# PJLab-ADG/neuralsim

Hardware: NVIDIA H100
Metric: Mrays/sec fwd+bwd (higher is better)
Workload: dtype f16

## Files before the change

### neuralsim_b200/csrc/color_tc.cu

```cuda
#include "fused_tc_common.cuh"
#include "sh_device.cuh"

namespace nsb {

struct ColorNetDev {
    DecoderDevTC dec;
    const __half *R1, *rb1, *R2, *rb2, *R3, *rb3;
    int rw, rin, n_appear;
    float fac[3];
};

constexpr int XW = 64;
constexpr int kTileBytes = kTile * XW * 2;
constexpr int kChunk = kTile * 16;

__host__ __device__ inline int ref_col(int k, int n_appear) {
    if (k < 32) return 22 + k;
    if (k < 35) return k - 32;
    if (k < 51) return 3 + (k - 35);
    if (k < 54) return 19 + (k - 51);
    if (k < 54 + n_appear) return k;
    return -1;
}


__device__ __forceinline__ void level_jacobian(const PLMeta &m, uint32_t p, const float (&xs)[3], const __half *__restrict__ grid,
                                               float (&J0)[3], float (&J1)[3]) {
    uint32_t cell[8];
    float w[8], fr[3], scale[3];
    level_cells3(m, p, xs, cell, w, fr, scale);
    const uint32_t *lp = level_cells_ptr(m, p, grid);
    float2 v[8];
#pragma unroll
    for (int c = 0; c < 8; ++c) {
        const uint32_t raw = ld_nc_u32(lp + cell[c]);
        v[c] = __half22float2(*reinterpret_cast<const __half2 *>(&raw));
    }
#pragma unroll
    for (int gd = 0; gd < 3; ++gd) {
        float a0 = 0.f, a1 = 0.f;
#pragma unroll
        for (int c = 0; c < 4; ++c) {
            float ww = scale[gd];
            int left = 0;
#pragma unroll
            for (int k = 0; k < 2; ++k) {
                const int d = k >= gd ? k + 1 : k;
                if (c & (1 << k)) { ww = __fmul_rn(ww, fr[d]); left += 1 << d; }
                else ww = __fmul_rn(ww, __fsub_rn(1.f, fr[d]));
            }
            const int right = left + (1 << gd);
            a0 = __fmaf_rn(ww, __fsub_rn(v[right].x, v[left].x), a0);
            a1 = __fmaf_rn(ww, __fsub_rn(v[right].y, v[left].y), a1);
        }
        J0[gd] = a0;
        J1[gd] = a1;
    }
}

__device__ __forceinline__ void unpack8(const uint4 &q, float (&v)[8]) {
    const __half2 *h = reinterpret_cast<const __half2 *>(&q);
#pragma unroll
    for (int i = 0; i < 4; ++i) { const float2 f = __half22float2(h[i]); v[2 * i] = f.x; v[2 * i + 1] = f.y; }
}

constexpr int kColorGatherU = 4;

constexpr int kColorBwdCtasPerSM = 2;

__global__ void __launch_bounds__(kTile)
k_color_fwd(const PLMeta m, const __half *__restrict__ grid, const ColorNetDev net, const PointSrc ps, const float *__restrict__ view_dirs,
            const float *__restrict__ h_appear, int64_t n, int max_level, float *__restrict__ sdf_out, float *__restrict__ nab_out,
            float *__restrict__ rgb_out, float *__restrict__ x_out, uint8_t *__restrict__ Zt, uint8_t *__restrict__ Xt,
            uint8_t *__restrict__ Y1t, uint8_t *__restrict__ Y2t, const OccCollect oc, const int64_t *__restrict__ n_dev) {
    n = eff_n(n, n_dev);
    extern __shared__ uint8_t dyn_smem[];
    uint8_t *tiles = reinterpret_cast<uint8_t *>((reinterpret_cast<uintptr_t>(dyn_smem) + 1023) & ~uintptr_t(1023));
    uint8_t *sX = tiles;
    uint8_t *sU = sX + kTileBytes;
    uint8_t *sW1 = sU + kTileBytes;
    uint8_t *sW1T = sW1 + HW * NF * 2;
    uint8_t *sR1 = sW1T + HW * NF * 2;
    uint8_t *sR2 = sR1 + XW * XW * 2;
    constexpr int kS = tc::acc_stride(64);
    float *acc = reinterpret_cast<float *>(sR2 + XW * XW * 2);
    __shared__ float sb1[HW], sW2[HW], srb1[XW], srb2[XW], sR3[3][XW];
    __shared__ float sb2, srb3[3];

    const int tid = threadIdx.x;
    stage_W1(net.dec, sW1, tid);
    stage_W1T(net.dec, sW1T, tid);
    for (int e = tid; e < XW * XW; e += kTile) {
        const int j = e % XW, k = e / XW;
        const int rc = ref_col(k, net.n_appear);
        const __half v1 = (j < net.rw && rc >= 0) ? net.R1[j * net.rin + rc] : __float2half_rn(0.f);
        const __half v2 = (j < net.rw && k < net.rw) ? net.R2[j * net.rw + k] : __float2half_rn(0.f);
        *reinterpret_cast<__half *>(sR1 + (k / 8) * (XW * 16) + j * 16 + (k % 8) * 2) = v1;
        *reinterpret_cast<__half *>(sR2 + (k / 8) * (XW * 16) + j * 16 + (k % 8) * 2) = v2;
    }
    stage_decoder_vectors(net.dec, sb1, sW2, &sb2, tid);
    if (tid < XW) {
        srb1[tid] = tid < net.rw ? __half2float(net.rb1[tid]) : 0.f;
        srb2[tid] = tid < net.rw ? __half2float(net.rb2[tid]) : 0.f;
#pragma unroll
        for (int k = 0; k < 3; ++k) sR3[k][tid] = tid < net.rw ? __half2float(net.R3[k * net.rw + tid]) : 0.f;
    }
    if (tid == 0) {
        for (int k = 0; k < 3; ++k) srb3[k] = __half2float(net.rb3[k]);
    }
    tc::fence_async_smem();
    __syncthreads();
    const uint32_t x_addr = tc::smem_u32(sX), u_addr = tc::smem_u32(sU), w1_addr = tc::smem_u32(sW1), w1t_addr = tc::smem_u32(sW1T);
    const uint32_t r1_addr = tc::smem_u32(sR1), r2_addr = tc::smem_u32(sR2);
    const SoftplusK spk(net.dec.beta);

    const int64_t n_tiles = (n + kTile - 1) / kTile;
    for (int64_t tile = blockIdx.x; tile < n_tiles; tile += gridDim.x) {
        const int64_t i = tile * kTile + tid;
        const bool valid = i < n;
        float xn[3], xs[3];
        int64_t ray;
        load_point(ps, ps.x == nullptr, i, valid, xn, xs, ray);
        gather_row_to_tile<kTile, kColorGatherU>(m, grid, xs, max_level, sX, tid);
        tc::fence_async_smem();
        __syncthreads();
        tc::mma_to_rows<64, 0, 0, NF / 16>(acc, kS, 0, tc::kmajor(x_addr, kTile), tc::kmajor(w1_addr, HW), false);
        __syncthreads();
        float out = 0.f;
        uint8_t *zt = Zt ? Zt + tile * kTileBytes : nullptr;
#pragma unroll 1
        for (int c = 0; c < HW / 8; ++c) {
            float z[8], uu[8];
            tc::acc_ld8(acc, kS, tid, c * 8, z);
#pragma unroll
            for (int j = 0; j < 8; ++j) {
                z[j] = r16(z[j] + sb1[c * 8 + j]);
                float a, s;
                softplus_as(z[j], spk, a, s);
                out = fmaf(r16(a), sW2[c * 8 + j], out);
                uu[j] = sW2[c * 8 + j] * s;
            }
            *reinterpret_cast<uint4 *>(sU + c * kChunk + tid * 16) = tc::pack8_f16(uu);
            if (zt) *reinterpret_cast<uint4 *>(zt + c * kChunk + tid * 16) = tc::pack8_f16(z);
        }
        const float sdf = r16(out + sb2);
        tc::fence_async_smem();
        __syncthreads();
        tc::mma_to_rows<32, 0, 0, HW / 16>(acc, kS, 0, tc::kmajor(u_addr, kTile), tc::kmajor(w1t_addr, NF), false);
        __syncthreads();
        float nacc[3] = {0.f, 0.f, 0.f};
#pragma unroll 1
        for (uint32_t g4 = 0; g4 < 4; ++g4) {
            float gg[8];
            tc::acc_ld8(acc, kS, tid, g4 * 8, gg);
#pragma unroll
            for (uint32_t q = 0; q < 4; ++q) {
                const uint32_t p = g4 * 4 + q;
                if ((int)m.level[p] <= max_level) {
                    float J0[3], J1[3];
                    level_jacobian(m, p, xs, grid, J0, J1);
                    const float g0 = r16(gg[2 * q]), g1 = r16(gg[2 * q + 1]);
#pragma unroll
                    for (int d = 0; d < 3; ++d) nacc[d] = __fmaf_rn(g0, J0[d], nacc[d]);
#pragma unroll
                    for (int d = 0; d < 3; ++d) nacc[d] = __fmaf_rn(g1, J1[d], nacc[d]);
                }
            }
        }
        float nab[3];
#pragma unroll
        for (int d = 0; d < 3; ++d) nab[d] = __fmul_rn(__fmul_rn(nacc[d], 0.5f), net.fac[d]);
        {
            float xr[32];
#pragma unroll
            for (int k = 0; k < 32; ++k) xr[k] = 0.f;
            xr[0] = xn[0]; xr[1] = xn[1]; xr[2] = xn[2];
            if (valid) {
                sh_basis(view_dirs[ray * 3], view_dirs[ray * 3 + 1], view_dirs[ray * 3 + 2], 4, xr + 3);
                if (h_appear) {
#pragma unroll
                    for (int k = 0; k < 8; ++k)
                        if (k < net.n_appear) xr[22 + k] = h_appear[ray * net.n_appear + k];
                }
            }
#pragma unroll
            for (int d = 0; d < 3; ++d) xr[19 + d] = fminf(fmaxf(nab[d], -1.f), 1.f);
            uint8_t *xt = Xt ? Xt + tile * kTileBytes : nullptr;
#pragma unroll
            for (int c = 0; c < 4; ++c) {
                float v8[8];
#pragma unroll
                for (int k = 0; k < 8; ++k) v8[k] = xr[c * 8 + k];
                const uint4 q = tc::pack8_f16(v8);
                *reinterpret_cast<uint4 *>(sX + (4 + c) * kChunk + tid * 16) = q;
                if (xt) {
                    *reinterpret_cast<uint4 *>(xt + (4 + c) * kChunk + tid * 16) = q;
                    *reinterpret_cast<uint4 *>(xt + c * kChunk + tid * 16) = *reinterpret_cast<const uint4 *>(sX + c * kChunk + tid * 16);
                }
            }
        }
        tc::fence_async_smem();
        __syncthreads();
        tc::mma_to_rows<64, 0, 0, XW / 16>(acc, kS, 0, tc::kmajor(x_addr, kTile), tc::kmajor(r1_addr, XW), false);
        __syncthreads();
        uint8_t *y1t = Y1t ? Y1t + tile * kTileBytes : nullptr;
#pragma unroll 1
        for (int c = 0; c < XW / 8; ++c) {
            float y[8];
            tc::acc_ld8(acc, kS, tid, c * 8, y);
#pragma unroll
            for (int j = 0; j < 8; ++j) y[j] = fmaxf(r16(y[j] + srb1[c * 8 + j]), 0.f);
            const uint4 q = tc::pack8_f16(y);
            *reinterpret_cast<uint4 *>(sU + c * kChunk + tid * 16) = q;
            if (y1t) *reinterpret_cast<uint4 *>(y1t + c * kChunk + tid * 16) = q;
        }
        tc::fence_async_smem();
        __syncthreads();
        tc::mma_to_rows<64, 0, 0, XW / 16>(acc, kS, 0, tc::kmajor(u_addr, kTile), tc::kmajor(r2_addr, XW), false);
        __syncthreads();
        float o3[3] = {0.f, 0.f, 0.f};
        uint8_t *y2t = Y2t ? Y2t + tile * kTileBytes : nullptr;
#pragma unroll 1
        for (int c = 0; c < XW / 8; ++c) {
            float y[8];
            tc::acc_ld8(acc, kS, tid, c * 8, y);
#pragma unroll
            for (int j = 0; j < 8; ++j) {
                y[j] = fmaxf(r16(y[j] + srb2[c * 8 + j]), 0.f);
#pragma unroll
                for (int k = 0; k < 3; ++k) o3[k] = fmaf(y[j], sR3[k][c * 8 + j], o3[k]);
            }
            if (y2t) *reinterpret_cast<uint4 *>(y2t + c * kChunk + tid * 16) = tc::pack8_f16(y);
        }
        if (valid) {
            sdf_out[i] = sdf;
            if (oc.pcl) occ_collect_point(oc, xs, sdf);
#pragma unroll
            for (int d = 0; d < 3; ++d) {
                nab_out[i * 3 + d] = nab[d];
                const float y3 = r16(o3[d] + srb3[d]);
                rgb_out[i * 3 + d] = r16(1.f / (1.f + expf(-y3)));
                if (x_out) x_out[i * 3 + d] = xn[d];
            }
        }
        __syncthreads();
    }
}

__global__ void __launch_bounds__(kTile, kColorBwdCtasPerSM)
k_color_rad_bwd(const ColorNetDev net, const uint8_t *__restrict__ Xt, const uint8_t *__restrict__ Y1t, const uint8_t *__restrict__ Y2t,
                const float *__restrict__ rgb, const float *__restrict__ g_rgb, int64_t n, float *__restrict__ dh_out,
                float *__restrict__ dR1, float *__restrict__ drb1, float *__restrict__ dR2, float *__restrict__ drb2,
                float *__restrict__ dR3, float *__restrict__ drb3, const int64_t *__restrict__ n_dev) {
    n = eff_n(n, n_dev);
    constexpr int NE = 80;
    extern __shared__ uint8_t dyn_smem[];
    uint8_t *tiles = reinterpret_cast<uint8_t *>((reinterpret_cast<uintptr_t>(dyn_smem) + 1023) & ~uintptr_t(1023));
    uint8_t *sT = tiles;
    uint8_t *sY1 = sT + 3 * kTileBytes;
    uint8_t *sXe = sY1 + kTile * NE * 2;
    uint8_t *sR2T = sXe + kTile * NE * 2;
    uint8_t *sR1h = sR2T + XW * XW * 2;
    __shared__ float sR3[3][XW];
    __shared__ float sdb3[3];
    __shared__ __align__(8) uint64_t mbar_ld;

    const int tid = threadIdx.x, lane = tid & 31;
    for (int e = tid; e < XW * XW; e += kTile) {
        const int i = e % XW, j = e / XW;
        const __half v = (j < net.rw && i < net.rw) ? net.R2[j * net.rw + i] : __float2half_rn(0.f);
        *reinterpret_cast<__half *>(sR2T + (j / 8) * (XW * 16) + i * 16 + (j % 8) * 2) = v;
    }
    for (int e = tid; e < NF * XW; e += kTile) {
        const int k = e % NF, j = e / NF;
        const __half v = j < net.rw ? net.R1[j * net.rin + 22 + k] : __float2half_rn(0.f);
        *reinterpret_cast<__half *>(sR1h + (j / 8) * (NF * 16) + k * 16 + (j % 8) * 2) = v;
    }
    if (tid < XW) {
#pragma unroll
        for (int k = 0; k < 3; ++k) sR3[k][tid] = tid < net.rw ? __half2float(net.R3[k * net.rw + tid]) : 0.f;
    }
    *reinterpret_cast<uint4 *>(sY1 + 8 * kChunk + tid * 16) = make_uint4(0x00003C00u, 0, 0, 0);
    *reinterpret_cast<uint4 *>(sY1 + 9 * kChunk + tid * 16) = make_uint4(0, 0, 0, 0);
    *reinterpret_cast<uint4 *>(sXe + 9 * kChunk + tid * 16) = make_uint4(0, 0, 0, 0);
    float xa[NE / 2], xb[NE / 2], x3[4];
#pragma unroll
    for (int k = 0; k < NE / 2; ++k) xa[k] = xb[k] = 0.f;
#pragma unroll
    for (int k = 0; k < 4; ++k) x3[k] = 0.f;
    if (tid == 0) {
        sdb3[0] = sdb3[1] = sdb3[2] = 0.f;
        tc::mbar_init(&mbar_ld, 1);
        tc::fence_mbar_init();
    }
    tc::fence_async_smem();
    __syncthreads();
    const uint32_t t_addr = tc::smem_u32(sT), y1_addr = tc::smem_u32(sY1), xe_addr = tc::smem_u32(sXe);
    const uint32_t r2t_addr = tc::smem_u32(sR2T), r1h_addr = tc::smem_u32(sR1h);
    uint32_t ld_phase = 0;
    bool first_tile = true;

    const int64_t n_tiles = (n + kTile - 1) / kTile;
    auto fetch = [&](int64_t tile) {
        tc::mbar_arrive_expect_tx(&mbar_ld, 3 * kTileBytes);
        tc::tma_load_bulk(sT + 2 * kTileBytes, Y2t + tile * kTileBytes, kTileBytes, &mbar_ld);
        tc::tma_load_bulk(sY1, Y1t + tile * kTileBytes, kTileBytes, &mbar_ld);
        tc::tma_load_bulk(sXe, Xt + tile * kTileBytes, kTileBytes, &mbar_ld);
    };
    if (tid == 0 && (int64_t)blockIdx.x < n_tiles) fetch(blockIdx.x);
    for (int64_t tile = blockIdx.x; tile < n_tiles; tile += gridDim.x) {
        const int64_t i = tile * kTile + tid;
        const bool valid = i < n;
        tc::mbar_wait(&mbar_ld, ld_phase);
        ld_phase ^= 1;
        float gy[3] = {0.f, 0.f, 0.f};
        if (valid && g_rgb) {
#pragma unroll
            for (int k = 0; k < 3; ++k) {
                const float y = rgb[i * 3 + k];
                gy[k] = r16(r16(g_rgb[i * 3 + k]) * ((1.f - y) * y));
            }
        }
        {
            float e8[8] = {1.f, gy[0], gy[1], gy[2], 0.f, 0.f, 0.f, 0.f};
            *reinterpret_cast<uint4 *>(sXe + 8 * kChunk + tid * 16) = tc::pack8_f16(e8);
        }
#pragma unroll
        for (int k = 0; k < 3; ++k) {
            const float sgy = warp_sum(gy[k]);
            if (lane == 0 && sgy != 0.f) atomicAdd(&sdb3[k], sgy);
        }
#pragma unroll 1
        for (int c = 0; c < 8; ++c) {
            float y2[8], d[8];
            unpack8(*reinterpret_cast<const uint4 *>(sT + 2 * kTileBytes + c * kChunk + tid * 16), y2);
#pragma unroll
            for (int j = 0; j < 8; ++j) {
                const float v = gy[0] * sR3[0][c * 8 + j] + gy[1] * sR3[1][c * 8 + j] + gy[2] * sR3[2][c * 8 + j];
                d[j] = y2[j] > 0.f ? v : 0.f;
            }
            *reinterpret_cast<uint4 *>(sT + c * kChunk + tid * 16) = tc::pack8_f16(d);
        }
        tc::fence_async_smem();
        __syncthreads();
        {
            float dy[2][XW / 2];
            tc::mma_m128<64, 0, 0, XW / 16>(dy, tc::kmajor(t_addr, kTile), tc::kmajor(r2t_addr, XW), false);
#pragma unroll
            for (int h = 0; h < 2; ++h)
#pragma unroll
                for (int c = 0; c < XW / 8; ++c)
#pragma unroll
                    for (int r = 0; r < 2; ++r) {
                        const uint32_t off = tc::pair_off<kTile>(h * 64 + tc::frag_row(r), tc::frag_col(c));
                        const float2 y1 = tc::ld_pair_f16(sY1, off);
                        tc::st_pair_f16(sT + kTileBytes, off, y1.x > 0.f ? dy[h][4 * c + 2 * r] : 0.f, y1.y > 0.f ? dy[h][4 * c + 2 * r + 1] : 0.f);
                    }
        }
        tc::fence_async_smem();
        __syncthreads();
        float dh[2][NF / 2];
        tc::mma_m128<32, 0, 0, XW / 16>(dh, tc::kmajor(t_addr + kTileBytes, kTile), tc::kmajor(r1h_addr, NF), false);
        tc::mma_m64<NE, 1, 1, kTile / 16>(xa, tc::mnmajor(t_addr, kTile), tc::mnmajor(y1_addr, kTile), true);
        tc::mma_m64<NE, 1, 1, kTile / 16>(xb, tc::mnmajor(t_addr + kTileBytes, kTile), tc::mnmajor(xe_addr, kTile), true);
        tc::mma_m64<8, 1, 1, kTile / 16>(x3, tc::mnmajor(t_addr + 2 * kTileBytes, kTile), tc::mnmajor(xe_addr + 8 * kChunk, kTile), true);
        first_tile = false;
        __syncthreads();
        if (tid == 0 && tile + gridDim.x < n_tiles) {
            tc::fence_async_smem();
            fetch(tile + gridDim.x);
        }
#pragma unroll
        for (int h = 0; h < 2; ++h)
#pragma unroll
            for (int r = 0; r < 2; ++r) {
                const int64_t row = tile * kTile + h * 64 + tc::frag_row(r);
                if (row < n) {
#pragma unroll
                    for (int c = 0; c < NF / 8; ++c)
                        *reinterpret_cast<float2 *>(dh_out + row * NF + tc::frag_col(c)) = make_float2(dh[h][4 * c + 2 * r], dh[h][4 * c + 2 * r + 1]);
                }
            }
    }
    if (!first_tile) {
#pragma unroll
        for (int r = 0; r < 2; ++r) {
            const int row = tc::frag_row(r);
            if (row >= net.rw) continue;
#pragma unroll
            for (int c = 0; c < NE / 8; ++c)
#pragma unroll
                for (int j = 0; j < 2; ++j) {
                    const int col = tc::frag_col(c) + j;
                    const float a = xa[4 * c + 2 * r + j], b = xb[4 * c + 2 * r + j];
                    if (col < XW) {
                        if (col < net.rw) atomicAdd(dR2 + row * net.rw + col, a);
                        const int rc = ref_col(col, net.n_appear);
                        if (rc >= 0) atomicAdd(dR1 + row * net.rin + rc, b);
                    } else if (col == XW) {
                        atomicAdd(drb2 + row, a);
                        atomicAdd(drb1 + row, b);
                    }
                }
#pragma unroll
            for (int j = 0; j < 2; ++j) {
                const int col = tc::frag_col(0) + j;
                if (col >= 1 && col <= 3) atomicAdd(dR3 + (col - 1) * net.rw + row, x3[2 * r + j]);
            }
        }
        if (tid < 3) atomicAdd(drb3 + tid, sdb3[tid]);
    }
}

__global__ void __launch_bounds__(kTile, kColorBwdCtasPerSM)
k_color_sdf_bwd(const PLMeta m, const __half *__restrict__ grid, const ColorNetDev net, const PointSrc ps, const uint8_t *__restrict__ Zt,
                const uint8_t *__restrict__ Xt, const float *__restrict__ g_nab, const float *__restrict__ g_sdf, const float *__restrict__ dh_r,
                int64_t n, int max_level, float *__restrict__ d_grid, float *__restrict__ d_W1, float *__restrict__ d_b1, float *__restrict__ d_W2,
                float *__restrict__ d_b2, const int64_t *__restrict__ n_dev) {
    n = eff_n(n, n_dev);
    constexpr int NX = 48;
    extern __shared__ uint8_t dyn_smem[];
    uint8_t *tiles = reinterpret_cast<uint8_t *>((reinterpret_cast<uintptr_t>(dyn_smem) + 1023) & ~uintptr_t(1023));
    uint8_t *sT = tiles;
    uint8_t *sHe = sT + 3 * kTileBytes;
    uint8_t *sGe = sHe + kTile * NX * 2;
    uint8_t *sW1 = sGe + kTile * NX * 2;
    uint8_t *sW1T = sW1 + HW * NF * 2;
    uint8_t *sZ = sW1T + NF * HW * 2;
    constexpr int kS = tc::acc_stride(2 * NF);
    float *stage = reinterpret_cast<float *>(sT);
    static_assert(kTile * kS * 4 <= 3 * kTileBytes, "the staged rows must fit in T");
    __shared__ float sW2[HW], sdsdf[kTile];
    __shared__ float sdb2;
    __shared__ __align__(8) uint64_t mbar_ld;

    const int tid = threadIdx.x, lane = tid & 31;
    stage_W1(net.dec, sW1, tid);
    stage_W1T(net.dec, sW1T, tid);
    stage_decoder_vectors(net.dec, nullptr, sW2, nullptr, tid);
    *reinterpret_cast<uint4 *>(sHe + 4 * kChunk + tid * 16) = make_uint4(0x00003C00u, 0, 0, 0);
    *reinterpret_cast<uint4 *>(sGe + 4 * kChunk + tid * 16) = make_uint4(0x00003C00u, 0, 0, 0);
    *reinterpret_cast<uint4 *>(sHe + 5 * kChunk + tid * 16) = make_uint4(0, 0, 0, 0);
    *reinterpret_cast<uint4 *>(sGe + 5 * kChunk + tid * 16) = make_uint4(0, 0, 0, 0);
    float wacc[NX / 2], vacc[4];
#pragma unroll
    for (int k = 0; k < NX / 2; ++k) wacc[k] = 0.f;
#pragma unroll
    for (int k = 0; k < 4; ++k) vacc[k] = 0.f;
    if (tid == 0) {
        sdb2 = 0.f;
        tc::mbar_init(&mbar_ld, 1);
        tc::fence_mbar_init();
    }
    tc::fence_async_smem();
    __syncthreads();
    const uint32_t t_addr = tc::smem_u32(sT), he_addr = tc::smem_u32(sHe), ge_addr = tc::smem_u32(sGe), w1_addr = tc::smem_u32(sW1),
                   w1t_addr = tc::smem_u32(sW1T);
    const SoftplusK spk(net.dec.beta);
    uint32_t ld_phase = 0;
    bool first_tile = true;

    const int64_t n_tiles = (n + kTile - 1) / kTile;
    auto fetch = [&](int64_t tile) {
        tc::mbar_arrive_expect_tx(&mbar_ld, kTileBytes + 4 * kChunk);
        tc::tma_load_bulk(sZ, Zt + tile * kTileBytes, kTileBytes, &mbar_ld);
        tc::tma_load_bulk(sHe, Xt + tile * kTileBytes, 4 * kChunk, &mbar_ld);
    };
    if (tid == 0 && (int64_t)blockIdx.x < n_tiles) fetch(blockIdx.x);
    for (int64_t tile = blockIdx.x; tile < n_tiles; tile += gridDim.x) {
        const int64_t i = tile * kTile + tid;
        const bool valid = i < n;
        float xn[3], xs[3];
        int64_t ray;
        load_point(ps, ps.x == nullptr, i, valid, xn, xs, ray);
        float gin[3] = {0.f, 0.f, 0.f};
        if (valid && g_nab) {
#pragma unroll
            for (int d = 0; d < 3; ++d) gin[d] = g_nab[i * 3 + d] * net.fac[d] * 0.5f;
        }
        const float dsdf = (valid && g_sdf) ? g_sdf[i] : 0.f;
        sdsdf[tid] = dsdf;
        tc::mbar_wait(&mbar_ld, ld_phase);
        ld_phase ^= 1;
#pragma unroll 1
        for (int c = 0; c < 8; ++c) {
            float z[8], uu[8];
            unpack8(*reinterpret_cast<const uint4 *>(sZ + c * kChunk + tid * 16), z);
#pragma unroll
            for (int j = 0; j < 8; ++j) {
                float a, s;
                softplus_as(z[j], spk, a, s);
                uu[j] = sW2[c * 8 + j] * s;
            }
            *reinterpret_cast<uint4 *>(sT + kTileBytes + c * kChunk + tid * 16) = tc::pack8_f16(uu);
        }
#pragma unroll 4
        for (uint32_t p = 0; p < 16; ++p) {
            uint32_t packed = 0;
            if ((int)m.level[p] <= max_level) {
                float J0[3], J1[3];
                level_jacobian(m, p, xs, grid, J0, J1);
                float a0 = 0.f, a1 = 0.f;
#pragma unroll
                for (int d = 0; d < 3; ++d) { a0 = __fmaf_rn(gin[d], J0[d], a0); a1 = __fmaf_rn(gin[d], J1[d], a1); }
                const __half2 h = __floats2half2_rn(a0, a1);
                packed = *reinterpret_cast<const uint32_t *>(&h);
            }
            *reinterpret_cast<uint32_t *>(sGe + (p >> 2) * kChunk + tid * 16 + (p & 3) * 4) = packed;
        }
        tc::fence_async_smem();
        __syncthreads();
        float gfr[2][NF / 2];
        {
            float du[2][HW / 2];
            tc::mma_m128<64, 0, 0, NF / 16>(du, tc::kmajor(ge_addr, kTile), tc::kmajor(w1_addr, HW), false);
            tc::mma_m128<32, 0, 0, HW / 16>(gfr, tc::kmajor(t_addr + kTileBytes, kTile), tc::kmajor(w1t_addr, NF), false);
#pragma unroll
            for (int h = 0; h < 2; ++h)
#pragma unroll
                for (int r = 0; r < 2; ++r) {
                    const int row = h * 64 + tc::frag_row(r);
                    const float ds = sdsdf[row];
#pragma unroll
                    for (int c = 0; c < HW / 8; ++c) {
                        const int col = tc::frag_col(c);
                        const uint32_t off = tc::pair_off<kTile>(row, col);
                        const float2 z2 = tc::ld_pair_f16(sZ, off);
                        float dz[2], vv[2];
#pragma unroll
                        for (int j = 0; j < 2; ++j) {
                            const float z = j ? z2.y : z2.x;
                            float a, s;
                            softplus_as(z, spk, a, s);
                            const float w2 = sW2[col + j], d = r16(du[h][4 * c + 2 * r + j]);
                            const float curv = (z * spk.k > spk.thr) ? 0.f : spk.beta * s * (1.f - s);
                            dz[j] = d * w2 * curv + ds * w2 * s;
                            vv[j] = d * s + ds * r16(a);
                        }
                        tc::st_pair_f16(sT, off, dz[0], dz[1]);
                        tc::st_pair_f16(sT + 2 * kTileBytes, off, vv[0], vv[1]);
                    }
                }
        }
        tc::fence_async_smem();
        __syncthreads();
        float dhz[2][NF / 2];
        tc::mma_m128<32, 0, 0, HW / 16>(dhz, tc::kmajor(t_addr, kTile), tc::kmajor(w1t_addr, NF), false);
        tc::mma_m64<NX, 1, 1, kTile / 16>(wacc, tc::mnmajor(t_addr, kTile), tc::mnmajor(he_addr, kTile), true);
        tc::mma_m64<NF, 1, 1, kTile / 16>(*reinterpret_cast<float(*)[NF / 2]>(wacc), tc::mnmajor(t_addr + kTileBytes, kTile), tc::mnmajor(ge_addr, kTile), true);
        tc::mma_m64<8, 1, 1, kTile / 16>(vacc, tc::mnmajor(t_addr + 2 * kTileBytes, kTile), tc::mnmajor(ge_addr + 4 * kChunk, kTile), true);
        first_tile = false;
        const float dsum = warp_sum(dsdf);
        if (lane == 0 && dsum != 0.f) atomicAdd(&sdb2, dsum);
        __syncthreads();
        if (tid == 0 && tile + gridDim.x < n_tiles) {
            tc::fence_async_smem();
            fetch(tile + gridDim.x);
        }
        tc::frag_store<NF>(gfr, stage, kS, 0);
        tc::frag_store<NF>(dhz, stage, kS, NF);
        __syncthreads();
#pragma unroll 1
        for (uint32_t g4 = 0; g4 < 4; ++g4) {
            float gg[8], hz[8];
            tc::acc_ld8(stage, kS, tid, g4 * 8, gg);
            tc::acc_ld8(stage, kS, tid, NF + g4 * 8, hz);
            if (valid && dh_r) {
                const float4 r0 = *reinterpret_cast<const float4 *>(dh_r + i * NF + g4 * 8), r1 = *reinterpret_cast<const float4 *>(dh_r + i * NF + g4 * 8 + 4);
                hz[0] += r0.x; hz[1] += r0.y; hz[2] += r0.z; hz[3] += r0.w; hz[4] += r1.x; hz[5] += r1.y; hz[6] += r1.z; hz[7] += r1.w;
            }
#pragma unroll
            for (uint32_t q = 0; q < 4; ++q) {
                const uint32_t p = g4 * 4 + q;
                if ((int)m.level[p] > max_level) continue;
                uint32_t cell[8];
                float w[8], fr[3], sc[3], ua[8], ub[8];
                level_cells3(m, p, xs, cell, w, fr, sc);
                const float g0 = valid ? r16(gg[2 * q]) : 0.f, g1 = valid ? r16(gg[2 * q + 1]) : 0.f;
                const float h0 = valid ? hz[2 * q] : 0.f, h1 = valid ? hz[2 * q + 1] : 0.f;
#pragma unroll
                for (int c = 0; c < 8; ++c) {
                    float wsum = 0.f;
#pragma unroll
                    for (int gd = 0; gd < 3; ++gd) {
                        float ww = __fmul_rn(sc[gd], gin[gd]);
#pragma unroll
                        for (int d = 0; d < 3; ++d) {
                            if (d == gd) continue;
                            ww = __fmul_rn(ww, (c & (1 << d)) ? fr[d] : __fsub_rn(1.f, fr[d]));
                        }
                        wsum += (c & (1 << gd)) ? ww : -ww;
                    }
                    ua[c] = g0 * wsum + h0 * w[c];
                    ub[c] = g1 * wsum + h1 * w[c];
                }
                bool issue = valid;
                if (level_mergeable(m, p)) issue = warp_merge_updates(cell_key3(m, p, xs), valid, ua, ub, lane);
                if (issue) {
                    float2 *gp = level_grad_ptr(m, p, d_grid);
#pragma unroll
                    for (int c = 0; c < 8; ++c) red_add2(gp + cell[c], ua[c], ub[c]);
                }
            }
        }
        __syncthreads();
    }
    if (!first_tile) {
#pragma unroll
        for (int r = 0; r < 2; ++r) {
            const int row = tc::frag_row(r);
            if (row >= net.dec.width) continue;
#pragma unroll
            for (int c = 0; c <= NF / 8; ++c)
#pragma unroll
                for (int j = 0; j < 2; ++j) {
                    const int col = tc::frag_col(c) + j;
                    if (col < NF) atomicAdd(d_W1 + row * NF + col, wacc[4 * c + 2 * r + j]);
                    else if (col == NF) atomicAdd(d_b1 + row, wacc[4 * c + 2 * r + j]);
                }
            if (tc::frag_col(0) == 0) atomicAdd(d_W2 + row, vacc[2 * r]);
        }
        if (tid == 0) atomicAdd(d_b2, sdb2);
    }
}

}

using namespace nsb;

namespace {
int make_net(const nsb_color_net *c, const nsb_lotd_meta *meta, PLMeta *m, ColorNetDev *d, const char *who) {
    const nsb_sdf_decoder dec{c->W1, c->b1, c->W2, c->b2, c->width, c->beta};
    if (int rc = make_decoder(meta, &dec, m, &d->dec, who)) return rc;
    NSB_REQUIRE(c->rad_width >= 1 && c->rad_width <= 64, "%s: radiance width must be <= 64", who);
    NSB_REQUIRE(c->n_appear >= 0 && c->n_appear <= 8 && c->rad_in == 54 + c->n_appear,
                "%s: radiance input must be [x(3), SH deg 4 (16), n(3), h(32), h_appear(<=8)]", who);
    d->R1 = (const __half *)c->R1; d->rb1 = (const __half *)c->rb1; d->R2 = (const __half *)c->R2; d->rb2 = (const __half *)c->rb2;
    d->R3 = (const __half *)c->R3; d->rb3 = (const __half *)c->rb3;
    d->rw = c->rad_width; d->rin = c->rad_in; d->n_appear = c->n_appear;
    for (int k = 0; k < 3; ++k) d->fac[k] = c->nablas_scale[k];
    return 0;
}
}

static int64_t n_tiles(int64_t n) { return (n + kTile - 1) / kTile; }

extern "C" int64_t nsb_color_tile_bytes(int64_t n) { return n_tiles(n) * (int64_t)kTileBytes; }

extern "C" int nsb_fused_color_fwd(const nsb_lotd_meta *meta, const void *params_half, const nsb_color_net *net, const float *x, const float *rays_o,
                                   const float *rays_d, const int64_t *ridx, const float *t, const float *view_dirs, const float *h_appear,
                                   int64_t n, int32_t max_level, float *sdf, float *nablas, float *rgb, float *x_out, void *act_z, void *act_x,
                                   void *act_y1, void *act_y2, const nsb_occ_collect *collect, void *stream) {
    const DevCounts dn = take_counts();
    if (n == 0) return 0;
    NSB_REQUIRE(meta && params_half && net && sdf && nablas && rgb && view_dirs, "nsb_fused_color_fwd: NULL argument");
    NSB_REQUIRE(x || (rays_o && rays_d && t), "nsb_fused_color_fwd: need x or (rays_o, rays_d, t)");
    NSB_REQUIRE((act_z && act_x && act_y1 && act_y2) || (!act_z && !act_x && !act_y1 && !act_y2), "nsb_fused_color_fwd: pass all four activation buffers or none");
    PLMeta m;
    ColorNetDev d;
    if (int rc = make_net(net, meta, &m, &d, "nsb_fused_color_fwd")) return rc;
    NSB_REQUIRE(d.n_appear == 0 || h_appear, "nsb_fused_color_fwd: h_appear is NULL but the net has %d appearance channels", d.n_appear);
    constexpr int kSmem = 2 * kTileBytes + 2 * HW * NF * 2 + 2 * XW * XW * 2 + kTile * tc::acc_stride(64) * 4 + 1024;
    opt_in_smem(k_color_fwd, kSmem);
    const PointSrc ps{x, rays_o, rays_d, t, ridx};
    k_color_fwd<<<persistent_grid(n_tiles(n), 2), kTile, kSmem, (cudaStream_t)stream>>>(m, (const __half *)params_half, d, ps, view_dirs, h_appear, n,
                                                                                        max_level < 0 ? -1 : max_level, sdf, nablas, rgb, x_out, (uint8_t *)act_z,
                                                                                        (uint8_t *)act_x, (uint8_t *)act_y1, (uint8_t *)act_y2,
                                                                                        occ_collect_of(collect), dn.a);
    return check_launch("nsb_fused_color_fwd");
}

extern "C" int nsb_fused_color_bwd(const nsb_lotd_meta *meta, const void *params_half, const nsb_color_net *net, const float *x, const float *rays_o,
                                   const float *rays_d, const int64_t *ridx, const float *t, int64_t n, int32_t max_level, const void *act_z,
                                   const void *act_x, const void *act_y1, const void *act_y2, const float *rgb, const float *g_sdf,
                                   const float *g_nablas, const float *g_rgb, float *dh_scratch, float *d_grid, float *d_W1, float *d_b1,
                                   float *d_W2, float *d_b2, float *d_R1, float *d_rb1, float *d_R2, float *d_rb2, float *d_R3, float *d_rb3,
                                   void *stream) {
    const DevCounts dn = take_counts();
    if (n == 0) return 0;
    NSB_REQUIRE(meta && params_half && net && act_z && act_x && act_y1 && act_y2 && rgb && dh_scratch, "nsb_fused_color_bwd: NULL argument");
    NSB_REQUIRE(d_grid && d_W1 && d_b1 && d_W2 && d_b2 && d_R1 && d_rb1 && d_R2 && d_rb2 && d_R3 && d_rb3, "nsb_fused_color_bwd: NULL gradient buffer");
    NSB_REQUIRE(x || (rays_o && rays_d && t), "nsb_fused_color_bwd: need x or (rays_o, rays_d, t)");
    PLMeta m;
    ColorNetDev d;
    if (int rc = make_net(net, meta, &m, &d, "nsb_fused_color_bwd")) return rc;
    cudaStream_t s = (cudaStream_t)stream;
    const float *dh = nullptr;
    if (g_rgb) {
        constexpr int kSmemR = 3 * kTileBytes + 2 * kTile * 80 * 2 + XW * XW * 2 + NF * XW * 2 + 1024;
        opt_in_smem(k_color_rad_bwd, kSmemR);
        if (int rc = require_ctas_per_sm(k_color_rad_bwd, kTile, kSmemR, kColorBwdCtasPerSM, "nsb_fused_color_bwd(radiance)")) return rc;
        k_color_rad_bwd<<<persistent_grid(n_tiles(n), kColorBwdCtasPerSM), kTile, kSmemR, s>>>(d, (const uint8_t *)act_x, (const uint8_t *)act_y1,
                                                                                               (const uint8_t *)act_y2, rgb, g_rgb, n, dh_scratch, d_R1,
                                                                                               d_rb1, d_R2, d_rb2, d_R3, d_rb3, dn.a);
        if (int rc = check_launch("nsb_fused_color_bwd(radiance)")) return rc;
        dh = dh_scratch;
    }
    constexpr int kSmemS = 3 * kTileBytes + 2 * kTile * 48 * 2 + 2 * HW * NF * 2 + kTileBytes + 1024;
    opt_in_smem(k_color_sdf_bwd, kSmemS);
    if (int rc = require_ctas_per_sm(k_color_sdf_bwd, kTile, kSmemS, kColorBwdCtasPerSM, "nsb_fused_color_bwd(sdf)")) return rc;
    const PointSrc ps{x, rays_o, rays_d, t, ridx};
    k_color_sdf_bwd<<<persistent_grid(n_tiles(n), kColorBwdCtasPerSM), kTile, kSmemS, s>>>(m, (const __half *)params_half, d, ps, (const uint8_t *)act_z, (const uint8_t *)act_x,
                                                                          g_nablas, g_sdf, dh, n, max_level < 0 ? -1 : max_level, d_grid, d_W1, d_b1, d_W2, d_b2, dn.a);
    return check_launch("nsb_fused_color_bwd(sdf)");
}
```

### neuralsim_b200/csrc/tc_util.cuh

```cuda
#pragma once
#include "nsb_common.cuh"

namespace nsb {
namespace tc {

__device__ __forceinline__ uint32_t smem_u32(const void *p) { return (uint32_t)__cvta_generic_to_shared(p); }

__device__ __forceinline__ uint64_t make_desc(uint32_t smem_addr, uint32_t lbo_bytes, uint32_t sbo_bytes) {
    uint64_t d = 0;
    d |= (uint64_t)((smem_addr >> 4) & 0x3FFF);
    d |= (uint64_t)((lbo_bytes >> 4) & 0x3FFF) << 16;
    d |= (uint64_t)((sbo_bytes >> 4) & 0x3FFF) << 32;
    return d;
}

struct Operand {
    uint32_t addr, lbo, sbo, kstep;
};
__device__ __forceinline__ Operand kmajor(uint32_t addr, int rows) { return Operand{addr, (uint32_t)rows * 16, 128, (uint32_t)rows * 32}; }
__device__ __forceinline__ Operand mnmajor(uint32_t addr, int rows) { return Operand{addr, 128, (uint32_t)rows * 16, 256}; }

template <int N, int TA, int TB>
struct Wgmma;
template <int TA, int TB>
struct Wgmma<8, TA, TB> {
    __device__ __forceinline__ static void mma(float (&d)[4], uint64_t a, uint64_t b, uint32_t acc) {
        asm volatile(
            "{\n\t.reg .pred p;\n\tsetp.ne.b32 p, %6, 0;\n\t"
            "wgmma.mma_async.sync.aligned.m64n8k16.f32.f16.f16 {%0, %1, %2, %3}, %4, %5, p, 1, 1, %7, %8;\n\t}\n"
            : "+f"(d[0]), "+f"(d[1]), "+f"(d[2]), "+f"(d[3])
            : "l"(a), "l"(b), "r"(acc), "n"(TA), "n"(TB));
    }
};
template <int TA, int TB>
struct Wgmma<32, TA, TB> {
    __device__ __forceinline__ static void mma(float (&d)[16], uint64_t a, uint64_t b, uint32_t acc) {
        asm volatile(
            "{\n\t.reg .pred p;\n\tsetp.ne.b32 p, %18, 0;\n\t"
            "wgmma.mma_async.sync.aligned.m64n32k16.f32.f16.f16 {%0, %1, %2, %3, %4, %5, %6, %7, %8, %9, %10, %11, %12, %13, %14, %15}, %16, %17, p, 1, 1, %19, %20;\n\t}\n"
            : "+f"(d[0]), "+f"(d[1]), "+f"(d[2]), "+f"(d[3]), "+f"(d[4]), "+f"(d[5]), "+f"(d[6]), "+f"(d[7]), "+f"(d[8]), "+f"(d[9]), "+f"(d[10]), "+f"(d[11]), "+f"(d[12]), "+f"(d[13]), "+f"(d[14]), "+f"(d[15])
            : "l"(a), "l"(b), "r"(acc), "n"(TA), "n"(TB));
    }
};
template <int TA, int TB>
struct Wgmma<40, TA, TB> {
    __device__ __forceinline__ static void mma(float (&d)[20], uint64_t a, uint64_t b, uint32_t acc) {
        asm volatile(
            "{\n\t.reg .pred p;\n\tsetp.ne.b32 p, %22, 0;\n\t"
            "wgmma.mma_async.sync.aligned.m64n40k16.f32.f16.f16 {%0, %1, %2, %3, %4, %5, %6, %7, %8, %9, %10, %11, %12, %13, %14, %15, %16, %17, %18, %19}, %20, %21, p, 1, 1, %23, %24;\n\t}\n"
            : "+f"(d[0]), "+f"(d[1]), "+f"(d[2]), "+f"(d[3]), "+f"(d[4]), "+f"(d[5]), "+f"(d[6]), "+f"(d[7]), "+f"(d[8]), "+f"(d[9]), "+f"(d[10]), "+f"(d[11]), "+f"(d[12]), "+f"(d[13]), "+f"(d[14]), "+f"(d[15]), "+f"(d[16]), "+f"(d[17]), "+f"(d[18]), "+f"(d[19])
            : "l"(a), "l"(b), "r"(acc), "n"(TA), "n"(TB));
    }
};
template <int TA, int TB>
struct Wgmma<48, TA, TB> {
    __device__ __forceinline__ static void mma(float (&d)[24], uint64_t a, uint64_t b, uint32_t acc) {
        asm volatile(
            "{\n\t.reg .pred p;\n\tsetp.ne.b32 p, %26, 0;\n\t"
            "wgmma.mma_async.sync.aligned.m64n48k16.f32.f16.f16 {%0, %1, %2, %3, %4, %5, %6, %7, %8, %9, %10, %11, %12, %13, %14, %15, %16, %17, %18, %19, %20, %21, %22, %23}, %24, %25, p, 1, 1, %27, %28;\n\t}\n"
            : "+f"(d[0]), "+f"(d[1]), "+f"(d[2]), "+f"(d[3]), "+f"(d[4]), "+f"(d[5]), "+f"(d[6]), "+f"(d[7]), "+f"(d[8]), "+f"(d[9]), "+f"(d[10]), "+f"(d[11]), "+f"(d[12]), "+f"(d[13]), "+f"(d[14]), "+f"(d[15]), "+f"(d[16]), "+f"(d[17]), "+f"(d[18]), "+f"(d[19]), "+f"(d[20]), "+f"(d[21]), "+f"(d[22]), "+f"(d[23])
            : "l"(a), "l"(b), "r"(acc), "n"(TA), "n"(TB));
    }
};
template <int TA, int TB>
struct Wgmma<64, TA, TB> {
    __device__ __forceinline__ static void mma(float (&d)[32], uint64_t a, uint64_t b, uint32_t acc) {
        asm volatile(
            "{\n\t.reg .pred p;\n\tsetp.ne.b32 p, %34, 0;\n\t"
            "wgmma.mma_async.sync.aligned.m64n64k16.f32.f16.f16 {%0, %1, %2, %3, %4, %5, %6, %7, %8, %9, %10, %11, %12, %13, %14, %15, %16, %17, %18, %19, %20, %21, %22, %23, %24, %25, %26, %27, %28, %29, %30, %31}, %32, %33, p, 1, 1, %35, %36;\n\t}\n"
            : "+f"(d[0]), "+f"(d[1]), "+f"(d[2]), "+f"(d[3]), "+f"(d[4]), "+f"(d[5]), "+f"(d[6]), "+f"(d[7]), "+f"(d[8]), "+f"(d[9]), "+f"(d[10]), "+f"(d[11]), "+f"(d[12]), "+f"(d[13]), "+f"(d[14]), "+f"(d[15]), "+f"(d[16]), "+f"(d[17]), "+f"(d[18]), "+f"(d[19]), "+f"(d[20]), "+f"(d[21]), "+f"(d[22]), "+f"(d[23]), "+f"(d[24]), "+f"(d[25]), "+f"(d[26]), "+f"(d[27]), "+f"(d[28]), "+f"(d[29]), "+f"(d[30]), "+f"(d[31])
            : "l"(a), "l"(b), "r"(acc), "n"(TA), "n"(TB));
    }
};
template <int TA, int TB>
struct Wgmma<80, TA, TB> {
    __device__ __forceinline__ static void mma(float (&d)[40], uint64_t a, uint64_t b, uint32_t acc) {
        asm volatile(
            "{\n\t.reg .pred p;\n\tsetp.ne.b32 p, %42, 0;\n\t"
            "wgmma.mma_async.sync.aligned.m64n80k16.f32.f16.f16 {%0, %1, %2, %3, %4, %5, %6, %7, %8, %9, %10, %11, %12, %13, %14, %15, %16, %17, %18, %19, %20, %21, %22, %23, %24, %25, %26, %27, %28, %29, %30, %31, %32, %33, %34, %35, %36, %37, %38, %39}, %40, %41, p, 1, 1, %43, %44;\n\t}\n"
            : "+f"(d[0]), "+f"(d[1]), "+f"(d[2]), "+f"(d[3]), "+f"(d[4]), "+f"(d[5]), "+f"(d[6]), "+f"(d[7]), "+f"(d[8]), "+f"(d[9]), "+f"(d[10]), "+f"(d[11]), "+f"(d[12]), "+f"(d[13]), "+f"(d[14]), "+f"(d[15]), "+f"(d[16]), "+f"(d[17]), "+f"(d[18]), "+f"(d[19]), "+f"(d[20]), "+f"(d[21]), "+f"(d[22]), "+f"(d[23]), "+f"(d[24]), "+f"(d[25]), "+f"(d[26]), "+f"(d[27]), "+f"(d[28]), "+f"(d[29]), "+f"(d[30]), "+f"(d[31]), "+f"(d[32]), "+f"(d[33]), "+f"(d[34]), "+f"(d[35]), "+f"(d[36]), "+f"(d[37]), "+f"(d[38]), "+f"(d[39])
            : "l"(a), "l"(b), "r"(acc), "n"(TA), "n"(TB));
    }
};

__device__ __forceinline__ void wgmma_fence() { asm volatile("wgmma.fence.sync.aligned;" ::: "memory"); }
__device__ __forceinline__ void wgmma_commit() { asm volatile("wgmma.commit_group.sync.aligned;" ::: "memory"); }
__device__ __forceinline__ void wgmma_wait_all() { asm volatile("wgmma.wait_group.sync.aligned 0;" ::: "memory"); }
__device__ __forceinline__ void fence_operand(float &r) { asm volatile("" : "+f"(r)::"memory"); }

template <int N, int TA, int TB, int KSTEPS>
__device__ __forceinline__ void mma_m128(float (&d)[2][N / 2], const Operand &a, const Operand &b, bool accumulate) {
#pragma unroll
    for (int h = 0; h < 2; ++h)
#pragma unroll
        for (int i = 0; i < N / 2; ++i) fence_operand(d[h][i]);
    wgmma_fence();
#pragma unroll
    for (int h = 0; h < 2; ++h)
#pragma unroll
        for (int ks = 0; ks < KSTEPS; ++ks)
            Wgmma<N, TA, TB>::mma(d[h], make_desc(a.addr + h * 8 * a.sbo + ks * a.kstep, a.lbo, a.sbo), make_desc(b.addr + ks * b.kstep, b.lbo, b.sbo),
                                  (ks > 0 || accumulate) ? 1u : 0u);
    wgmma_commit();
    wgmma_wait_all();
#pragma unroll
    for (int h = 0; h < 2; ++h)
#pragma unroll
        for (int i = 0; i < N / 2; ++i) fence_operand(d[h][i]);
}

template <int N, int TA, int TB, int KSTEPS>
__device__ __forceinline__ void mma_m64(float (&d)[N / 2], const Operand &a, const Operand &b, bool accumulate) {
#pragma unroll
    for (int i = 0; i < N / 2; ++i) fence_operand(d[i]);
    wgmma_fence();
#pragma unroll
    for (int ks = 0; ks < KSTEPS; ++ks)
        Wgmma<N, TA, TB>::mma(d, make_desc(a.addr + ks * a.kstep, a.lbo, a.sbo), make_desc(b.addr + ks * b.kstep, b.lbo, b.sbo),
                              (ks > 0 || accumulate) ? 1u : 0u);
    wgmma_commit();
    wgmma_wait_all();
#pragma unroll
    for (int i = 0; i < N / 2; ++i) fence_operand(d[i]);
}

__device__ __forceinline__ int frag_row(int i) { return (threadIdx.x >> 5) * 16 + ((threadIdx.x & 31) >> 2) + 8 * i; }
__device__ __forceinline__ int frag_col(int c) { return c * 8 + 2 * (threadIdx.x & 3); }
template <int R>
__device__ __forceinline__ uint32_t pair_off(int row, int col) { return (uint32_t)((col >> 3) * (R * 16) + row * 16 + (col & 7) * 2); }
__device__ __forceinline__ float2 ld_pair_f16(const uint8_t *tile, uint32_t off) {
    return __half22float2(*reinterpret_cast<const __half2 *>(tile + off));
}
__device__ __forceinline__ void st_pair_f16(uint8_t *tile, uint32_t off, float a, float b) {
    *reinterpret_cast<__half2 *>(tile + off) = __floats2half2_rn(a, b);
}

constexpr int acc_stride(int cols) { return cols + 4; }

template <int N>
__device__ __forceinline__ void frag_store(const float (&d)[2][N / 2], float *acc, int stride, int col0) {
    const int w = threadIdx.x >> 5, l = threadIdx.x & 31;
#pragma unroll
    for (int h = 0; h < 2; ++h)
#pragma unroll
        for (int c = 0; c < N / 8; ++c)
#pragma unroll
            for (int i = 0; i < 2; ++i) {
                const int row = h * 64 + w * 16 + (l >> 2) + 8 * i, col = col0 + c * 8 + 2 * (l & 3);
                *reinterpret_cast<float2 *>(acc + row * stride + col) = make_float2(d[h][4 * c + 2 * i], d[h][4 * c + 2 * i + 1]);
            }
}
template <int N>
__device__ __forceinline__ void frag_load(float (&d)[2][N / 2], const float *acc, int stride, int col0) {
    const int w = threadIdx.x >> 5, l = threadIdx.x & 31;
#pragma unroll
    for (int h = 0; h < 2; ++h)
#pragma unroll
        for (int c = 0; c < N / 8; ++c)
#pragma unroll
            for (int i = 0; i < 2; ++i) {
                const int row = h * 64 + w * 16 + (l >> 2) + 8 * i, col = col0 + c * 8 + 2 * (l & 3);
                const float2 v = *reinterpret_cast<const float2 *>(acc + row * stride + col);
                d[h][4 * c + 2 * i] = v.x;
                d[h][4 * c + 2 * i + 1] = v.y;
            }
}
template <int N, int TA, int TB, int KSTEPS>
__device__ __forceinline__ void mma_to_rows(float *acc, int stride, int col0, const Operand &a, const Operand &b, bool accumulate) {
    float d[2][N / 2];
    if (accumulate) frag_load<N>(d, acc, stride, col0);
    else {
#pragma unroll
        for (int h = 0; h < 2; ++h)
#pragma unroll
            for (int i = 0; i < N / 2; ++i) d[h][i] = 0.f;
    }
    mma_m128<N, TA, TB, KSTEPS>(d, a, b, accumulate);
    frag_store<N>(d, acc, stride, col0);
}

__device__ __forceinline__ void acc_ld8(const float *acc, int stride, int row, int col, float (&v)[8]) {
    const float4 a = *reinterpret_cast<const float4 *>(acc + row * stride + col), b = *reinterpret_cast<const float4 *>(acc + row * stride + col + 4);
    v[0] = a.x; v[1] = a.y; v[2] = a.z; v[3] = a.w; v[4] = b.x; v[5] = b.y; v[6] = b.z; v[7] = b.w;
}

__device__ __forceinline__ void mbar_init(uint64_t *bar, uint32_t count) {
    asm volatile("mbarrier.init.shared::cta.b64 [%0], %1;" ::"r"(smem_u32(bar)), "r"(count) : "memory");
}
__device__ __forceinline__ void mbar_wait(uint64_t *bar, uint32_t parity) {
    asm volatile(
        "{\n\t.reg .pred p;\n\tWAIT_%=:\n\t"
        "mbarrier.try_wait.parity.shared::cta.b64 p, [%0], %1;\n\t"
        "@p bra DONE_%=;\n\tbra WAIT_%=;\n\tDONE_%=:\n\t}\n" ::"r"(smem_u32(bar)),
        "r"(parity)
        : "memory");
}

__device__ __forceinline__ void mbar_arrive_expect_tx(uint64_t *bar, uint32_t bytes) {
    asm volatile("mbarrier.arrive.expect_tx.shared::cta.b64 _, [%0], %1;" ::"r"(smem_u32(bar)), "r"(bytes) : "memory");
}
__device__ __forceinline__ void tma_load_bulk(void *smem_dst, const void *gmem_src, uint32_t bytes, uint64_t *bar) {
    asm volatile("cp.async.bulk.shared::cluster.global.mbarrier::complete_tx::bytes [%0], [%1], %2, [%3];" ::"r"(smem_u32(smem_dst)), "l"(gmem_src),
                 "r"(bytes), "r"(smem_u32(bar))
                 : "memory");
}

__device__ __forceinline__ void fence_async_smem() { asm volatile("fence.proxy.async.shared::cta;" ::: "memory"); }
__device__ __forceinline__ void fence_mbar_init() { asm volatile("fence.mbarrier_init.release.cluster;" ::: "memory"); }

__device__ __forceinline__ uint4 pack8_f16(const float (&v)[8]) {
    __half2 h0 = __floats2half2_rn(v[0], v[1]), h1 = __floats2half2_rn(v[2], v[3]);
    __half2 h2 = __floats2half2_rn(v[4], v[5]), h3 = __floats2half2_rn(v[6], v[7]);
    uint4 q;
    q.x = *reinterpret_cast<uint32_t *>(&h0); q.y = *reinterpret_cast<uint32_t *>(&h1);
    q.z = *reinterpret_cast<uint32_t *>(&h2); q.w = *reinterpret_cast<uint32_t *>(&h3);
    return q;
}

template <int R, int K>
__device__ __forceinline__ void store_row_f16(uint8_t *tile, int r, const float *vals) {
#pragma unroll
    for (int c = 0; c < K / 8; ++c) {
        __half2 h0 = __floats2half2_rn(vals[c * 8 + 0], vals[c * 8 + 1]);
        __half2 h1 = __floats2half2_rn(vals[c * 8 + 2], vals[c * 8 + 3]);
        __half2 h2 = __floats2half2_rn(vals[c * 8 + 4], vals[c * 8 + 5]);
        __half2 h3 = __floats2half2_rn(vals[c * 8 + 6], vals[c * 8 + 7]);
        uint4 q;
        q.x = *reinterpret_cast<uint32_t *>(&h0);
        q.y = *reinterpret_cast<uint32_t *>(&h1);
        q.z = *reinterpret_cast<uint32_t *>(&h2);
        q.w = *reinterpret_cast<uint32_t *>(&h3);
        *reinterpret_cast<uint4 *>(tile + c * (R * 16) + r * 16) = q;
    }
}

}
}
```

### neuralsim_b200/fields/fused_color.py

```python
from __future__ import annotations

import ctypes

import torch
from torch import autograd

from .. import _lib as L


class _FusedColor(autograd.Function):
    @staticmethod
    def forward(ctx, model, pts, view_dirs, h_appear, max_level, keep, collect, *params):
        grid16, net, _held = model._fused_color_state()
        ridx, t, rays_o, rays_d = pts
        n, dev = t.numel(), t.device
        meta = model.implicit_surface.encoding.meta
        sdf = torch.empty(n, dtype=torch.float32, device=dev)
        nab = torch.empty(n, 3, dtype=torch.float32, device=dev)
        rgb = torch.empty(n, 3, dtype=torch.float32, device=dev)
        x = torch.empty(n, 3, dtype=torch.float32, device=dev)
        acts = None
        if keep:
            acts = torch.empty(4, int(L.lib().nsb_color_tile_bytes(L.c_i64(n))), dtype=torch.uint8, device=dev)
        ap = [L.ptr(acts[k]) if keep else None for k in range(4)]
        with L.KERNEL_TIMER.time("fused_color_fwd", n):
            L.check(L.lib().nsb_fused_color_fwd(meta.c_ref, L.ptr(grid16, "f16"), ctypes.byref(net), None, L.ptr(rays_o, "f32"), L.ptr(rays_d, "f32"),
                                                L.ptr(ridx, "i64"), L.ptr(t, "f32"), L.ptr(view_dirs, "f32"), L.ptr(h_appear, "f32", allow_none=True),
                                                L.c_i64(n), L.c_i32(max_level), L.ptr(sdf), L.ptr(nab), L.ptr(rgb), L.ptr(x), *ap,
                                                ctypes.byref(collect) if collect is not None else None, L.stream_ptr()),
                    "fused_color_fwd")
        ctx.model, ctx.pts, ctx.max_level, ctx.n = model, pts, max_level, n
        ctx.held = (grid16, net, _held, acts, rgb)
        ctx.shapes = [p.shape for p in params]
        ctx.set_materialize_grads(False)
        ctx.mark_non_differentiable(x)
        return sdf, nab, rgb, x

    @staticmethod
    @autograd.function.once_differentiable
    def backward(ctx, g_sdf, g_nab, g_rgb, _gx):
        grid16, net, _held, acts, rgb = ctx.held
        if acts is None:
            raise RuntimeError("fused_color: backward through a forward that ran without grad")
        dev, n = rgb.device, ctx.n
        meta = ctx.model.implicit_surface.encoding.meta
        sizes = [int(torch.Size(s).numel()) for s in ctx.shapes[1:]]
        small = torch.zeros(sum(sizes), dtype=torch.float32, device=dev)
        grads, o = [torch.zeros(ctx.shapes[0], dtype=torch.float32, device=dev)], 0
        for sh, k in zip(ctx.shapes[1:], sizes):
            grads.append(small[o:o + k].view(sh))
            o += k
        if g_sdf is None and g_nab is None and g_rgb is None:
            return (None,) * 7 + tuple(grads)
        ridx, t, rays_o, rays_d = ctx.pts
        c = lambda g: None if g is None else g.contiguous().float()
        g_sdf, g_nab, g_rgb = c(g_sdf), c(g_nab), c(g_rgb)
        dh = torch.empty(n, 32, dtype=torch.float32, device=dev)
        with L.KERNEL_TIMER.time("fused_color_bwd", n):
            L.check(L.lib().nsb_fused_color_bwd(meta.c_ref, L.ptr(grid16, "f16"), ctypes.byref(net), None, L.ptr(rays_o, "f32"), L.ptr(rays_d, "f32"),
                                                L.ptr(ridx, "i64"), L.ptr(t, "f32"), L.c_i64(n), L.c_i32(ctx.max_level), L.ptr(acts[0]), L.ptr(acts[1]),
                                                L.ptr(acts[2]), L.ptr(acts[3]), L.ptr(rgb), L.ptr(g_sdf, allow_none=True), L.ptr(g_nab, allow_none=True),
                                                L.ptr(g_rgb, allow_none=True), L.ptr(dh), *[L.ptr(g) for g in grads], L.stream_ptr()),
                    "fused_color_bwd")
        return (None,) * 7 + tuple(grads)


def fused_color(model, ridx, t, rays_o, rays_d, view_dirs, h_appear=None, *, nablas_has_grad=True, collect=None):
    s, r = model.implicit_surface, model.radiance_net.blocks.layers
    d = s.decoder.layers
    params = (s.encoding.flattened_params, d[0].weight, d[0].bias, d[1].weight, d[1].bias, r[0].weight, r[0].bias, r[1].weight, r[1].bias,
              r[2].weight, r[2].bias)
    pts = (ridx.reshape(-1).contiguous().long(), t.detach().reshape(-1).contiguous().float(), rays_o.detach().contiguous().float(),
           rays_d.detach().contiguous().float())
    keep = torch.is_grad_enabled() and any(p.requires_grad for p in params)
    ha = None if h_appear is None else h_appear.detach().contiguous().float()
    sdf, nab, rgb, x = _FusedColor.apply(model, pts, view_dirs.detach().contiguous().float(), ha, s._ml(model.max_level), keep, collect, *params)
    if not nablas_has_grad:
        nab = nab.detach()
    return dict(sdf=sdf, nablas=nab, rgb=rgb, x=x)
```

### neuralsim_b200/graphics/neus_static.py

```python
from __future__ import annotations

import ctypes

import torch
import torch.nn.functional as F

from .. import _lib as L
from .raysample import batch_sample_step_linear
from .pack_ops import get_pack_infos_from_batch
from . import neus_fused as NF

__all__ = ["render_static", "StaticFrame", "CNT_SLOTS"]

CNT_SLOTS = dict(n_rays=0, pairs=2, marched_raw=3, hit_raw=4, kept_raw=6, kept_rays_raw=7, nonzero=9, marched=12, hit=13, fine0=14,
                 boundary=18, kept=19, overflow=20, kept_rays=21, merged0=22, rays_if_kept_fits=26, row_len=27)
_NULL = ctypes.c_void_p(0)
MARCH_ONEPASS = "auto"
MARCH_ONEPASS_MAX_BYTES = 64 << 20


def march_onepass(n_rays, max_steps):
    if MARCH_ONEPASS == "0":
        return False
    return MARCH_ONEPASS == "1" or 4 * int(n_rays) * int(max_steps) <= MARCH_ONEPASS_MAX_BYTES


def _slot(cnt, k):
    return ctypes.c_void_p(cnt.data_ptr() + 8 * k)


def _call(fn, what, cnt, k0, k1, *args):
    lib = L.lib()
    lib.nsb_bind_device_counts(_slot(cnt, k0), _slot(cnt, k1) if k1 is not None else _NULL)
    try:
        rc = fn(*args)
    finally:
        lib.nsb_bind_device_counts(_NULL, _NULL)
    L.check(rc, what)


def _scan(counts, cnt, slot, *, first=None, info2=None, index=None, pack=None, src=None, nz_src=None, ws=None):
    if ws is None:
        ws = torch.zeros(NF._scan_ws_bytes(), dtype=torch.uint8, device=counts.device)
    P = L.ptr
    L.check(L.lib().nsb_scan_counts(P(counts, "i32"), L.c_i64(counts.shape[0]), P(first, allow_none=True), P(info2, allow_none=True),
                                    P(index, allow_none=True), P(pack, allow_none=True), P(src, "i64", allow_none=True), P(nz_src, allow_none=True),
                                    _slot(cnt, slot), None, L.c_i64(0), P(ws), L.stream_ptr()), "scan_counts")


def _query_counts(cnt, phase, n_coarse1, num_fine, march_cap, kept_cap):
    nf = (ctypes.c_int32 * max(len(num_fine), 1))(*[int(n) for n in num_fine])
    L.check(L.lib().nsb_query_counts(ctypes.c_void_p(cnt.data_ptr()), L.c_i32(phase), L.c_i32(n_coarse1), nf, L.c_i32(len(num_fine)),
                                     L.c_i64(march_cap), L.c_i64(kept_cap), L.stream_ptr()), "query_counts")


def _sdf_launch(meta, grid16, dec, rays_o, rays_d, t, sdf, *, ridx=None, packs=None, ml, collect, cnt, slot, timer="lotd_gather"):
    P = L.ptr
    mode = 2 if packs is not None else 1
    with L.KERNEL_TIMER.time(timer, t.numel()):
        _call(L.lib().nsb_fused_sdf_collect, "fused_sdf", cnt, slot, None,
              meta.c_ref, P(grid16, "f16"), ctypes.byref(dec), None, P(rays_o, "f32"), P(rays_d, "f32"),
              P(ridx, "i64") if mode == 1 else None, P(t, "f32"), L.c_i64(t.numel()),
              P(packs[0], "i64") if mode == 2 else None, P(packs[1], "i64", allow_none=True) if mode == 2 else None,
              P(packs[2], "i64", allow_none=True) if mode == 2 and len(packs) > 2 else None,
              L.c_i64(packs[0].shape[0] if mode == 2 else 0), L.c_i32(mode), L.c_i32(ml), P(sdf),
              ctypes.byref(collect) if collect is not None else None, L.stream_ptr())
    return sdf


def _block_order(rays_inds, via, n_rays, cnt, slot):
    n = rays_inds.shape[0] if via is None else via.shape[0]
    order = torch.empty(n, dtype=torch.int64, device=rays_inds.device)
    _call(L.lib().nsb_ray_block_order, "ray_block_order", cnt, slot, None, L.ptr(rays_inds, "i64"), L.ptr(via, "i64", allow_none=True), L.c_i64(n),
          L.c_i64(n_rays), _slot(cnt, CNT_SLOTS["pairs"]), _slot(cnt, CNT_SLOTS["row_len"]), L.ptr(order), L.stream_ptr())
    return order


class _StaticSDF(torch.autograd.Function):

    @staticmethod
    def forward(ctx, st, ridx, t, packs, count_slot, grid, W1, b1, W2, b2):
        sdf = torch.empty(t.numel(), dtype=torch.float32, device=t.device)
        _sdf_launch(st.meta, st.grid16, st.dec, st.rays_o, st.rays_d, t, sdf, ridx=ridx if packs is None else None, packs=packs, ml=st.ml,
                    collect=st.collect, cnt=st.cnt, slot=count_slot, timer="fused_sdf_fwd")
        ctx.st, ctx.ridx, ctx.t = st, ridx, t
        ctx.shapes = (grid.shape, W1.shape, b1.shape, W2.shape, b2.shape)
        return sdf

    @staticmethod
    @torch.autograd.function.once_differentiable
    def backward(ctx, d_sdf):
        st, dev = ctx.st, d_sdf.device
        gs, w1s, b1s, w2s, b2s = ctx.shapes
        d_grid = torch.zeros(gs, dtype=torch.float32, device=dev)
        ks = [int(torch.Size(x).numel()) for x in (w1s, b1s, w2s, b2s)]
        small = torch.zeros(sum(ks), dtype=torch.float32, device=dev)
        d_W1, d_b1 = small[:ks[0]].view(w1s), small[ks[0]:ks[0] + ks[1]].view(b1s)
        d_W2, d_b2 = small[ks[0] + ks[1]:ks[0] + ks[1] + ks[2]].view(w2s), small[ks[0] + ks[1] + ks[2]:].view(b2s)
        d_sdf = d_sdf.contiguous().float()
        n = d_sdf.numel()
        P, cnt = L.ptr, st.cnt
        flag = torch.empty(n, dtype=torch.int32, device=dev)
        _call(L.lib().nsb_flag_nonzero, "flag_nonzero", cnt, CNT_SLOTS["boundary"], None, P(d_sdf, "f32"), L.c_i64(n), P(flag), L.stream_ptr())
        keep = torch.empty(n, dtype=torch.int64, device=dev)
        _scan(flag, cnt, CNT_SLOTS["nonzero"], index=keep, ws=st.ws[3])
        with L.KERNEL_TIMER.time("fused_sdf_bwd", n):
            _call(L.lib().nsb_fused_sdf_bwd_indexed, "fused_sdf_bwd", cnt, CNT_SLOTS["nonzero"], None,
                  st.meta.c_ref, P(st.grid16, "f16"), ctypes.byref(st.dec), None, P(st.rays_o, "f32"), P(st.rays_d, "f32"), P(ctx.ridx, "i64"),
                  P(ctx.t, "f32"), P(d_sdf, "f32"), P(keep, "i64"), L.c_i64(n), L.c_i32(st.ml), P(d_grid), P(d_W1), P(d_b1), P(d_W2), P(d_b2),
                  L.stream_ptr())
        return None, None, None, None, None, d_grid, d_W1, d_b1, d_W2, d_b2


class _StaticAlpha(torch.autograd.Function):

    @staticmethod
    def forward(ctx, sdf, inv_s, pack_infos, cnt, early_stop_eps, alpha_thre):
        sdf_c, inv_c = sdf.detach().contiguous().float(), inv_s.detach().contiguous().float().reshape(1)
        Pn, dev = pack_infos.shape[0], sdf_c.device
        alpha = torch.empty_like(sdf_c)
        sel = torch.empty(sdf_c.shape[0], dtype=torch.bool, device=dev)
        steps = torch.empty(Pn, dtype=torch.int32, device=dev)
        P = L.ptr
        _call(L.lib().nsb_neus_alpha_forward, "neus_alpha_forward", cnt, CNT_SLOTS["n_rays"], None, P(sdf_c, "f32"), P(pack_infos, "i64"), L.c_i64(Pn),
              P(inv_c, "f32"), L.c_f32(early_stop_eps), L.c_f32(alpha_thre), P(alpha), P(sel), P(steps), L.stream_ptr())
        ctx.save_for_backward(sdf_c, inv_c, pack_infos)
        ctx.cnt, ctx.inv_shape = cnt, inv_s.shape
        ctx.mark_non_differentiable(sel, steps)
        return alpha, sel, steps

    @staticmethod
    def backward(ctx, g_alpha, _gs, _gn):
        sdf_c, inv_c, pack_infos = ctx.saved_tensors
        g = g_alpha.contiguous().float()
        d_sdf = torch.empty_like(sdf_c)
        d_inv = torch.zeros(1, device=sdf_c.device, dtype=torch.float32)
        P = L.ptr
        _call(L.lib().nsb_neus_alpha_backward, "neus_alpha_backward", ctx.cnt, CNT_SLOTS["n_rays"], None, P(sdf_c, "f32"), P(pack_infos, "i64"),
              L.c_i64(pack_infos.shape[0]), P(inv_c, "f32"), P(g, "f32"), P(d_sdf), P(d_inv), L.stream_ptr())
        return (d_sdf if ctx.needs_input_grad[0] else None, d_inv.reshape(ctx.inv_shape) if ctx.needs_input_grad[1] else None, None, None, None, None)


class _StaticGather(torch.autograd.Function):

    @staticmethod
    def forward(ctx, src, pidx, gathered, cnt):
        ctx.save_for_backward(pidx)
        ctx.n, ctx.cnt = src.shape[0], cnt
        return gathered

    @staticmethod
    def backward(ctx, g):
        pidx, = ctx.saved_tensors
        g = g.contiguous().float()
        d = torch.zeros(ctx.n, dtype=torch.float32, device=g.device)
        P = L.ptr
        _call(L.lib().nsb_scatter_f32, "scatter_f32", ctx.cnt, CNT_SLOTS["kept"], None, P(g, "f32"), P(pidx, "i64"), L.c_i64(pidx.shape[0]), P(d), L.stream_ptr())
        return d, None, None, None


class _StaticColor(torch.autograd.Function):

    @staticmethod
    def forward(ctx, st, ridx, t, view_dirs, h_appear, keep_acts, *params):
        n, dev = t.numel(), t.device
        sdf = torch.empty(n, dtype=torch.float32, device=dev)
        nab = torch.empty(n, 3, dtype=torch.float32, device=dev)
        rgb = torch.empty(n, 3, dtype=torch.float32, device=dev)
        x = torch.empty(n, 3, dtype=torch.float32, device=dev)
        acts = torch.empty(4, int(L.lib().nsb_color_tile_bytes(L.c_i64(n))), dtype=torch.uint8, device=dev) if keep_acts else None
        ap = [L.ptr(acts[k]) if keep_acts else None for k in range(4)]
        P = L.ptr
        with L.KERNEL_TIMER.time("fused_color_fwd", n):
            _call(L.lib().nsb_fused_color_fwd, "fused_color_fwd", st.cnt, CNT_SLOTS["kept"], None,
                  st.meta.c_ref, P(st.grid16, "f16"), ctypes.byref(st.net), None, P(st.rays_o, "f32"), P(st.rays_d, "f32"), P(ridx, "i64"), P(t, "f32"),
                  P(view_dirs, "f32"), P(h_appear, "f32", allow_none=True), L.c_i64(n), L.c_i32(st.ml), P(sdf), P(nab), P(rgb), P(x), *ap,
                  ctypes.byref(st.collect) if st.collect is not None else None, L.stream_ptr())
        ctx.st, ctx.ridx, ctx.t, ctx.n = st, ridx, t, n
        ctx.held = (acts, rgb)
        ctx.shapes = [p.shape for p in params]
        ctx.set_materialize_grads(False)
        ctx.mark_non_differentiable(x)
        return sdf, nab, rgb, x

    @staticmethod
    @torch.autograd.function.once_differentiable
    def backward(ctx, g_sdf, g_nab, g_rgb, _gx):
        acts, rgb = ctx.held
        if acts is None:
            raise RuntimeError("static colour query: backward through a forward that ran without grad")
        st, dev, n = ctx.st, rgb.device, ctx.n
        sizes = [int(torch.Size(s).numel()) for s in ctx.shapes[1:]]
        small = torch.zeros(sum(sizes), dtype=torch.float32, device=dev)
        grads, o = [torch.zeros(ctx.shapes[0], dtype=torch.float32, device=dev)], 0
        for sh, k in zip(ctx.shapes[1:], sizes):
            grads.append(small[o:o + k].view(sh))
            o += k
        if g_sdf is None and g_nab is None and g_rgb is None:
            return (None,) * 6 + tuple(grads)
        c = lambda g: None if g is None else g.contiguous().float()
        g_sdf, g_nab, g_rgb = c(g_sdf), c(g_nab), c(g_rgb)
        dh = torch.empty(n, 32, dtype=torch.float32, device=dev)
        P = L.ptr
        with L.KERNEL_TIMER.time("fused_color_bwd", n):
            _call(L.lib().nsb_fused_color_bwd, "fused_color_bwd", st.cnt, CNT_SLOTS["kept"], None,
                  st.meta.c_ref, P(st.grid16, "f16"), ctypes.byref(st.net), None, P(st.rays_o, "f32"), P(st.rays_d, "f32"), P(ctx.ridx, "i64"),
                  P(ctx.t, "f32"), L.c_i64(n), L.c_i32(st.ml), P(acts[0]), P(acts[1]), P(acts[2]), P(acts[3]), P(rgb), P(g_sdf, allow_none=True),
                  P(g_nab, allow_none=True), P(g_rgb, allow_none=True), P(dh), *[P(g) for g in grads], L.stream_ptr())
        return (None,) * 6 + tuple(grads)


class _StaticComposite(torch.autograd.Function):

    @staticmethod
    def forward(ctx, alpha, t, rgb, nablas, pack_infos, ray_index, n_rays, cnt, normalize_depth, early_stop_eps, alpha_thre):
        a, tt = alpha.detach().contiguous().float(), t.detach().contiguous().float()
        r = None if rgb is None else rgb.detach().contiguous().float()
        nb = None if nablas is None else nablas.detach().contiguous().float()
        Pn, dev = pack_infos.shape[0], a.device
        vw = torch.empty_like(a)
        cols = 2 + (3 if r is not None else 0) + (3 if nb is not None else 0)
        buf = torch.zeros(cols * n_rays, device=dev)
        mask, depth = buf[:n_rays], buf[n_rays:2 * n_rays]
        rgb_o = buf[2 * n_rays:5 * n_rays].view(n_rays, 3) if r is not None else None
        o3 = 5 * n_rays if r is not None else 2 * n_rays
        nab_o = buf[o3:o3 + 3 * n_rays].view(n_rays, 3) if nb is not None else None
        P = L.ptr
        _call(L.lib().nsb_composite_forward, "composite_forward", cnt, CNT_SLOTS["kept_rays"], None, P(a, "f32"), P(tt, "f32"), P(r, "f32", allow_none=True),
              P(nb, "f32", allow_none=True), P(pack_infos, "i64"), L.c_i64(Pn), L.c_f32(early_stop_eps), L.c_f32(alpha_thre),
              ctypes.c_int(1 if normalize_depth else 0), P(ray_index, "i64"), P(vw), P(mask), P(depth), P(rgb_o, allow_none=True),
              P(nab_o, allow_none=True), L.stream_ptr())
        ctx.save_for_backward(a, tt, r, nb, vw, pack_infos, mask, depth, ray_index)
        ctx.cfg = (normalize_depth, early_stop_eps, alpha_thre, cnt)
        ctx.set_materialize_grads(False)
        empty = a.new_empty(0)
        return vw, mask, depth, (rgb_o if rgb_o is not None else empty), (nab_o if nab_o is not None else empty)

    @staticmethod
    def backward(ctx, g_vw, g_mask, g_depth, g_rgb, g_nab):
        a, tt, r, nb, vw, pack_infos, mask, depth, ray_index = ctx.saved_tensors
        normalize_depth, eps, thre, cnt = ctx.cfg

        def opt(g, present=True):
            return None if (g is None or not present) else g.contiguous().float()
        g_vw, g_mask, g_depth = opt(g_vw), opt(g_mask), opt(g_depth)
        g_rgb, g_nab = opt(g_rgb, r is not None), opt(g_nab, nb is not None)
        d_alpha = torch.empty_like(a)
        d_rgb = torch.empty_like(r) if r is not None else None
        d_nab = torch.empty_like(nb) if nb is not None else None
        P = L.ptr
        _call(L.lib().nsb_composite_backward, "composite_backward", cnt, CNT_SLOTS["kept_rays"], None,
              P(a, "f32"), P(tt, "f32"), P(r, allow_none=True), P(nb, allow_none=True), P(vw, "f32"), P(pack_infos, "i64"), L.c_i64(pack_infos.shape[0]),
              L.c_f32(eps), L.c_f32(thre), ctypes.c_int(1 if normalize_depth else 0), P(mask), P(depth), P(g_mask, allow_none=True),
              P(g_depth, allow_none=True), P(g_rgb, allow_none=True), P(g_nab, allow_none=True), P(g_vw, allow_none=True), P(ray_index, "i64"),
              P(d_alpha), P(d_rgb, allow_none=True), P(d_nab, allow_none=True), L.stream_ptr())
        return (d_alpha, None, d_rgb, d_nab) + (None,) * 7


class _State:
    __slots__ = ("meta", "grid16", "dec", "net", "held", "rays_o", "rays_d", "ml", "collect", "cnt", "ws")


def _fp16_images(model):
    s, b = model.implicit_surface, model.radiance_net.blocks.layers
    d = s.decoder.layers
    ps = [s.encoding.flattened_params, d[0].weight, d[0].bias, d[1].weight, d[1].bias, b[0].weight, b[0].bias, b[1].weight, b[1].bias, b[2].weight, b[2].bias]
    t = [torch.empty(p.shape, dtype=torch.half, device=p.device) for p in ps]
    with torch.no_grad():
        t[0].copy_(ps[0].detach())
        torch._foreach_copy_(t[1:], [p.detach() for p in ps[1:]])
    dec = L.SdfDecoderC(t[1].data_ptr(), t[2].data_ptr(), t[3].data_ptr(), t[4].data_ptr(), d[0].out_features, float(d[0].activation.beta))
    r3 = s.radius3d_original
    fk = (r3.data_ptr(), r3._version, float(s.sdf_scale))
    if getattr(model, "_fac_cache", (None,))[0] != fk:
        model._fac_cache = (fk, (s.sdf_scale / r3).float().tolist())
    net = L.ColorNetC(*[x.data_ptr() for x in t[1:]], d[0].out_features, b[0].out_features, b[0].in_features, b[0].in_features - 54,
                      float(d[0].activation.beta), (ctypes.c_float * 3)(*model._fac_cache[1]))
    return t, dec, net, ps


def static_supported(model, cfg):
    qp = dict(model.ray_query_cfg.get("query_param", {}) or {})
    occ = getattr(getattr(model, "accel", None), "occ", None)
    return (getattr(model, "_color_fusable", lambda: False)() and model.use_view_dirs and occ is not None and occ.occ_grid.dim() == 3
            and occ.occ_grid.numel() * 4 // 32 <= 96 * 1024 and qp.get("num_coarse", 0) > 0 and len(qp.get("upsample_inv_s_factors", (1, 4, 16))) <= 4
            and qp.get("coarse_step_cfg", {}).get("step_mode", "linear") == "linear" and (cfg.get("with_rgb", True) or cfg.get("with_normal", True)))


def render_static(model, rays_o, rays_d, rays_h_appear=None, *, near=None, far=None, march_cap, kept_cap, coherent=False, with_rgb=True, with_normal=True,
                  perturb=False, training=None, depth_use_normalized_vw=True, cnt=None):
    P, lib = L.ptr, L.lib()
    if perturb:
        raise RuntimeError("render_static: perturb=True is not built (random streams of capacity-sized draws differ from the reference's); "
                           "use the host-sized path (SingleVolumeRenderer.render)")
    training = model.training if training is None else training
    R, dev = rays_o.shape[0], rays_o.device
    qp = dict(model.ray_query_cfg.get("query_param", {}) or {})
    nc1 = int(qp["num_coarse"]) + 1
    factors = list(qp.get("upsample_inv_s_factors", (1, 4, 16)))
    n_stage = len(factors)
    num_fine = qp.get("num_fine", 8)
    num_fine = [num_fine] * n_stage if isinstance(num_fine, int) else list(num_fine)
    num_fine = [n // 2 * 2 + 1 for n in num_fine]
    nf_tot = int(sum(num_fine))
    upsample_inv_s = qp.get("upsample_inv_s", 64.) / model.upsample_s_divisor
    use_est = bool(qp.get("upsample_use_estimate_alpha", False))
    nablas_has_grad = bool(qp.get("nablas_has_grad", False))
    mc = dict(qp.get("march_cfg", {}))
    fac = mc.pop("step_size_factor", 1.0)
    step_size, dt_gamma = mc.get("step_size", 1e-3) * fac, mc.get("dt_gamma", 0.0) * fac
    max_steps, max_step_size = int(mc.get("max_steps", 512)), mc.get("max_step_size", 1e10)
    march_cap, kept_cap = int(march_cap), int(kept_cap)
    S_cap = R * (nc1 + nf_tot)
    if cnt is None:
        cnt = torch.zeros(32, dtype=torch.int64, device=dev)
    else:
        cnt.zero_()
    st = _State()
    st.cnt = cnt
    wsb = (NF._scan_ws_bytes() + 255) // 256 * 256
    st.ws = torch.zeros(4, wsb, dtype=torch.uint8, device=dev)
    with torch.no_grad():
        t16, st.dec, st.net, masters = _fp16_images(model)
        st.held, st.grid16 = t16, t16[0]
        st.meta = model.implicit_surface.encoding.meta
        st.ml = model.implicit_surface._ml(model.max_level)
        st.collect = model.accel.occ.collect_struct() if training else None
        sp = model.space
        if getattr(sp, "_host_cr", None) is None or sp._host_cr[0] != (sp.aabb.data_ptr(), sp.aabb._version):
            c, r = sp.center.tolist(), sp.radius3d.tolist()
            sp._host_cr = ((sp.aabb.data_ptr(), sp.aabb._version), (ctypes.c_float * 3)(*c), (ctypes.c_float * 3)(*r))
        o_n, d_n = torch.empty(R, 3, device=dev), torch.empty(R, 3, device=dev)
        nr, fr = torch.empty(R, device=dev), torch.empty(R, device=dev)
        flag = torch.empty(R, dtype=torch.int32, device=dev)
        L.check(lib.nsb_ray_test_aabb(P(rays_o.contiguous(), "f32"), P(rays_d.contiguous(), "f32"), L.c_i64(R), sp._host_cr[1], sp._host_cr[2],
                                      ctypes.c_int(0 if near is None else 1), L.c_f32(0. if near is None else near),
                                      ctypes.c_int(0 if far is None else 1), L.c_f32(0. if far is None else far), P(o_n), P(d_n), P(nr), P(fr), P(flag),
                                      _slot(cnt, CNT_SLOTS["pairs"]), _slot(cnt, CNT_SLOTS["row_len"]), L.stream_ptr()), "ray_test_aabb")
        rays_inds = torch.empty(R, dtype=torch.int64, device=dev)
        _scan(flag, cnt, CNT_SLOTS["n_rays"], index=rays_inds, ws=st.ws[0])
        order_b = _block_order(rays_inds, None, R, cnt, CNT_SLOTS["n_rays"]) if coherent else None
        ha = rays_h_appear.detach().contiguous().float() if (rays_h_appear is not None and model.use_h_appear) else None
        if ha is None and model.use_h_appear:
            ha = torch.zeros(R, model.radiance_net.blocks.layers[0].in_features - 54, device=dev)
        n_ha = ha.shape[1] if ha is not None else 0
        rbuf = torch.zeros(R * (8 + n_ha), device=dev)
        o_c, d_c = rbuf[:3 * R].view(R, 3), rbuf[3 * R:6 * R].view(R, 3)
        n_c, f_c = rbuf[6 * R:7 * R], rbuf[7 * R:8 * R]
        ha_c = rbuf[8 * R:].view(R, n_ha) if ha is not None else None
        _call(lib.nsb_gather_rays, "gather_rays", cnt, CNT_SLOTS["n_rays"], None, P(rays_inds, "i64"), L.c_i64(R), P(o_n), P(d_n), P(nr), P(fr), P(o_c), P(d_c),
              P(n_c), P(f_c), P(ha, allow_none=True), P(ha_c, allow_none=True), L.c_i32(0 if ha is None else ha.shape[1]), L.stream_ptr())
        st.rays_o, st.rays_d = o_c, d_c
        view_dirs = (d_c / d_c.norm(dim=-1).clamp_min(1.0e-10).unsqueeze(-1)).contiguous()
        coarse = batch_sample_step_linear(n_c, f_c, nc1, prefix_shape=[R], perturb=perturb).contiguous()
        occ_grid = model.accel.occ.occ_grid
        res = occ_grid.shape[-3:]
        g8 = occ_grid.contiguous().view(torch.uint8)
        bits = torch.empty((occ_grid.numel() + 31) // 32, dtype=torch.int32, device=dev)
        L.check(lib.nsb_pack_occ_bits(P(g8, "u8"), L.c_i64(occ_grid.numel()), P(bits), L.stream_ptr()), "pack_occ_bits")
        roi = torch.tensor([-1, -1, -1, 1, 1, 1], dtype=torch.float32, device=dev) if getattr(model, "_static_roi", None) is None else model._static_roi
        model._static_roi = roi
        margs = (L.c_i64(R), P(o_c, "f32"), P(d_c, "f32"), P(n_c, "f32"), P(f_c, "f32"), P(roi, "f32"), None, L.c_i32(res[0]), L.c_i32(res[1]), L.c_i32(res[2]),
                 P(g8, "u8"), L.c_f32(step_size), L.c_f32(max_step_size), L.c_f32(dt_gamma), ctypes.c_uint32(max_steps))
        num_steps = torch.empty(R, dtype=torch.int32, device=dev)
        rec_t = torch.empty(R * max_steps, dtype=torch.float32, device=dev) if march_onepass(R, max_steps) else None
        with L.KERNEL_TIMER.time("march", R):
            if rec_t is not None:
                _call(lib.nsb_ray_marching_record, "ray_marching_record", cnt, CNT_SLOTS["n_rays"], None, L.c_i64(R), P(o_c, "f32"), P(d_c, "f32"), P(n_c, "f32"),
                      P(f_c, "f32"), P(roi, "f32"), L.c_i32(res[0]), L.c_i32(res[1]), L.c_i32(res[2]), P(g8, "u8"), L.c_f32(step_size), L.c_f32(max_step_size),
                      L.c_f32(dt_gamma), ctypes.c_uint32(max_steps), P(num_steps), P(rec_t), P(bits), L.stream_ptr())
            else:
                _call(lib.nsb_ray_marching_listed, "ray_marching", cnt, CNT_SLOTS["n_rays"], None, *margs, None, P(num_steps), None, None, None, None, None, None,
                      L.c_i64(0), P(bits), L.stream_ptr())
        info2 = torch.empty(R, 2, dtype=torch.int32, device=dev)
        ridx_hit = torch.empty(R, dtype=torch.int64, device=dev)
        pack_infos = torch.empty(R, 2, dtype=torch.int64, device=dev)
        _scan(num_steps, cnt, CNT_SLOTS["marched_raw"], info2=info2, index=ridx_hit, pack=pack_infos, ws=st.ws[1])
        _query_counts(cnt, 0, nc1, num_fine, march_cap, kept_cap)
        depth = torch.empty(march_cap, dtype=torch.float32, device=dev)
        ridx32 = torch.empty(march_cap, dtype=torch.int32, device=dev)
        with L.KERNEL_TIMER.time("march", R):
            if rec_t is not None:
                _call(lib.nsb_march_compact, "march_compact", cnt, CNT_SLOTS["hit"], None, P(rec_t, "f32"), ctypes.c_uint32(max_steps), P(info2, "i32"),
                      P(ridx_hit, "i64"), L.c_i64(R), P(depth), P(ridx32), L.stream_ptr())
            else:
                _call(lib.nsb_ray_marching_listed, "ray_marching", cnt, CNT_SLOTS["hit"], None, *margs, P(info2), None, P(depth), None, P(ridx32), None, None,
                      P(ridx_hit, "i64"), L.c_i64(R), P(bits), L.stream_ptr())
        ridx = ridx32.long()
        from . import neus as GN
        fine_stages = None
        if GN.use_persistent_upsample(R):
            fine_all, _ovf = NF.upsample_rays(st.meta, st.grid16, st.dec, ridx_hit, pack_infos, depth, o_c, d_c, [upsample_inv_s * f for f in factors], num_fine,
                                              max_level=st.ml, max_steps=max_steps, use_estimate_alpha=use_est, collect=st.collect, count=(cnt, CNT_SLOTS["hit"]))
            factors_loop = []
        else:
            factors_loop = factors
        sdf = torch.empty(march_cap if factors_loop else 1, dtype=torch.float32, device=dev)
        if factors_loop:
            fine_stages = []
            order_f = _block_order(rays_inds, ridx_hit, R, cnt, CNT_SLOTS["hit"]) if coherent and n_stage > 1 else None
            _sdf_launch(st.meta, st.grid16, st.dec, o_c, d_c, depth, sdf, ridx=ridx, ml=st.ml, collect=st.collect, cnt=cnt, slot=CNT_SLOTS["marched"])
        for i, factor in enumerate(factors_loop):
            cdf = torch.empty(march_cap, dtype=torch.float32, device=dev)
            _call(lib.nsb_neus_upsample_cdf, "neus_upsample_cdf", cnt, CNT_SLOTS["hit"], None, P(sdf, "f32"), P(depth, "f32"), P(pack_infos, "i64"), L.c_i64(R),
                  L.c_f32(upsample_inv_s * factor), ctypes.c_int(1 if use_est else 0), L.c_f32(1e-4), L.c_f32(0.0), P(cdf), L.stream_ptr())
            nf = num_fine[i]
            fine = torch.empty(R, nf, dtype=torch.float32, device=dev)
            u = NF._U_CACHE.get((nf, dev))
            if u is None:
                u = NF._U_CACHE[(nf, dev)] = torch.linspace(0., 1., nf + 2, device=dev, dtype=torch.float32)[1:-1].contiguous()
            _call(lib.nsb_packed_invert_cdf_shared_u, "packed_invert_cdf_shared_u", cnt, CNT_SLOTS["hit"], None, P(depth, "f32"), P(cdf, "f32"), P(u, "f32"),
                  P(pack_infos, "i64"), L.c_i64(R), L.c_i32(nf), P(fine), L.stream_ptr())
            fine_stages.append(fine)
            if i < n_stage - 1:
                sdf_fine = torch.empty(R * nf, dtype=torch.float32, device=dev)
                if coherent:
                    _sdf_launch(st.meta, st.grid16, st.dec, o_c, d_c, fine.view(-1), sdf_fine, packs=(get_pack_infos_from_batch(R, nf, device=dev), ridx_hit, order_f),
                                ml=st.ml, collect=st.collect, cnt=cnt, slot=CNT_SLOTS["hit"])
                else:
                    _sdf_launch(st.meta, st.grid16, st.dec, o_c, d_c, fine.view(-1), sdf_fine, ridx=ridx_hit.unsqueeze(-1).expand(R, nf).reshape(-1).contiguous(),
                                ml=st.ml, collect=st.collect, cnt=cnt, slot=CNT_SLOTS["fine0"] + i)
                dep_m = torch.empty(march_cap, dtype=torch.float32, device=dev)
                sdf_m = torch.empty(march_cap, dtype=torch.float32, device=dev)
                pim = torch.empty_like(pack_infos)
                _call(lib.nsb_merge_sorted_vals, "merge_sorted_vals", cnt, CNT_SLOTS["hit"], None, P(depth, "f32"), P(sdf, "f32"), P(pack_infos, "i64"),
                      P(fine, "f32"), P(sdf_fine, "f32"), L.c_i64(R), L.c_i32(nf), P(dep_m), P(sdf_m), P(pim), L.stream_ptr())
                depth, sdf, pack_infos = dep_m, sdf_m, pim
        if fine_stages is not None:
            fine_all = (torch.cat(fine_stages, dim=-1) if n_stage > 1 else fine_stages[0]).contiguous()
        d1 = torch.empty(S_cap, dtype=torch.float32, device=dev)
        mid = torch.empty(S_cap, dtype=torch.float32, device=dev)
        ridx_all = torch.empty(S_cap, dtype=torch.int64, device=dev)
        pinfo = torch.empty(R, 2, dtype=torch.int64, device=dev)
        rl = (ctypes.c_int32 * n_stage)(*num_fine)
        _call(lib.nsb_assemble_boundary, "assemble_boundary", cnt, CNT_SLOTS["n_rays"], CNT_SLOTS["hit"], P(coarse, "f32"), L.c_i64(R), L.c_i32(nc1),
              P(ridx_hit, "i64"), L.c_i64(R), P(fine_all, "f32"), L.c_i32(nf_tot), rl, L.c_i32(n_stage), P(d1), P(mid), P(ridx_all), P(pinfo), L.stream_ptr())
    s, b = model.implicit_surface, model.radiance_net.blocks.layers
    dl = s.decoder.layers
    sdf_b = _StaticSDF.apply(st, ridx_all, d1, (pinfo, None, order_b) if coherent else None, CNT_SLOTS["n_rays"] if coherent else CNT_SLOTS["boundary"],
                             s.encoding.flattened_params, dl[0].weight, dl[0].bias, dl[1].weight, dl[1].bias)
    inv_s = model.forward_inv_s()
    if not isinstance(inv_s, torch.Tensor):
        inv_s = torch.tensor(float(inv_s), device=dev)
    alpha, sel, steps = _StaticAlpha.apply(sdf_b, inv_s, pinfo, cnt, 1e-4, 0.0)
    with torch.no_grad():
        first = torch.empty(R, dtype=torch.int32, device=dev)
        nidx = torch.empty(R, dtype=torch.int64, device=dev)
        pinfo_kept = torch.empty(R, 2, dtype=torch.int64, device=dev)
        rays_inds_hit = torch.empty(R, dtype=torch.int64, device=dev)
        _scan(steps, cnt, CNT_SLOTS["kept_raw"], first=first, index=nidx, pack=pinfo_kept, src=rays_inds, nz_src=rays_inds_hit, ws=st.ws[2])
        _query_counts(cnt, 1, nc1, num_fine, march_cap, kept_cap)
        pidx, ridx_k = torch.empty(kept_cap, dtype=torch.int64, device=dev), torch.empty(kept_cap, dtype=torch.int64, device=dev)
        t_k, alpha_c = torch.empty(kept_cap, dtype=torch.float32, device=dev), torch.empty(kept_cap, dtype=torch.float32, device=dev)
        _call(lib.nsb_compact_samples, "compact_samples", cnt, CNT_SLOTS["rays_if_kept_fits"], None, P(sel.view(torch.uint8), "u8"), P(pinfo, "i64"), P(first, "i32"),
              P(steps, "i32"), L.c_i64(R), P(ridx_all, "i64"), P(mid, "f32"), P(alpha.detach(), "f32"), P(pidx), P(ridx_k), P(t_k), P(alpha_c), L.stream_ptr())
    alpha_k = _StaticGather.apply(alpha, pidx, alpha_c, cnt) if alpha.requires_grad else alpha_c
    params = (s.encoding.flattened_params, dl[0].weight, dl[0].bias, dl[1].weight, dl[1].bias, b[0].weight, b[0].bias, b[1].weight, b[1].bias,
              b[2].weight, b[2].bias)
    keep_acts = torch.is_grad_enabled() and any(p.requires_grad for p in params)
    _sdf_k, nab, rgb, x = _StaticColor.apply(st, ridx_k, t_k, view_dirs, ha_c, keep_acts, *params)
    if not nablas_has_grad:
        nab = nab.detach()
    nab_i = nab if with_normal else None
    if nab_i is not None and not training:
        nab_i = F.normalize(nab_i.clamp(-1, 1), dim=-1)
    vw, m, d, c, nn_ = _StaticComposite.apply(alpha_k, t_k, rgb if with_rgb else None, nab_i, pinfo_kept, rays_inds_hit, R, cnt,
                                              bool(depth_use_normalized_vw), 1e-4, 0.0)
    rendered = dict(mask_volume=m, depth_volume=d)
    if with_rgb:
        rendered["rgb_volume"] = c
    if with_normal:
        rendered["normals_volume"] = nn_
    buffers = dict(opacity_alpha=alpha_k, t=t_k, rgb=rgb, nablas=nab, net_x=x, vw=vw, pack_infos_hit=pinfo_kept, rays_inds_hit=rays_inds_hit, ridx=ridx_k,
                   pack_infos_boundary=pinfo, march_pack_infos=pack_infos)
    return rendered, cnt, buffers


def sliced_volume_buffer(buffers, cnt):
    c = cnt.tolist()
    K, Pu = c[CNT_SLOTS["kept"]], c[CNT_SLOTS["kept_rays"]]
    if c[CNT_SLOTS["overflow"]]:
        raise RuntimeError(f"static step: arena overflow (flags {c[CNT_SLOTS['overflow']]}: 1 = marched samples, 2 = kept samples)")
    if K == 0:
        return dict(type="empty", rays_inds_hit=[])
    vb = dict(type="packed", rays_inds_hit=buffers["rays_inds_hit"][:Pu], pack_infos_hit=buffers["pack_infos_hit"][:Pu])
    for k in ("opacity_alpha", "t", "rgb", "nablas", "net_x", "vw"):
        vb[k] = buffers[k][:K]
    return vb


class StaticFrame:

    def __init__(self, model, n_rays, loss_fn=None, *, near=None, far=None, with_rgb=True, with_normal=True, slack=1.5, march_cap=None, kept_cap=None,
                 coherent=None, use_graph=True, zero_grads=False, h_appear_dim=None, pre_hook=None):
        self.model, self.n_rays, self.loss_fn = model, int(n_rays), loss_fn
        self.near, self.far, self.with_rgb, self.with_normal, self.slack = near, far, with_rgb, with_normal, float(slack)
        self.march_cap, self.kept_cap, self.coherent = march_cap, kept_cap, coherent
        self.use_graph, self.zero_grads, self.pre_hook = use_graph, zero_grads, pre_hook
        dev = model.device
        self.device = dev
        self.rays_o = torch.zeros(self.n_rays, 3, device=dev)
        self.rays_d = torch.zeros(self.n_rays, 3, device=dev)
        na = h_appear_dim if h_appear_dim is not None else (model.radiance_net.blocks.layers[0].in_features - 54 if model.use_h_appear else 0)
        self.h_appear = torch.zeros(self.n_rays, na, device=dev) if na > 0 else None
        self.cnt = torch.zeros(32, dtype=torch.int64, device=dev)
        self.graph, self.loss, self.rendered, self.buffers, self._occ_captured = None, None, None, None, None
        self.captures = 0

    @torch.no_grad()
    def _probe(self):
        from ..renderer import SingleVolumeRenderer
        r = SingleVolumeRenderer(dict(near=self.near, far=self.far, with_rgb=self.with_rgb, with_normal=self.with_normal))
        r.train(self.model.training)
        out = r.ray_query(self.model, self.rays_o, self.rays_d, self.h_appear, return_buffer=True, return_details=True)
        det, vb = out.get("details", {}), out["volume_buffer"]
        qp = dict(self.model.ray_query_cfg.get("query_param", {}) or {})
        nf = qp.get("num_fine", 8)
        nf = [nf] * len(qp.get("upsample_inv_s_factors", (1, 4, 16))) if isinstance(nf, int) else list(nf)
        nf = [n // 2 * 2 + 1 for n in nf]
        M = int(det["march.num_per_ray"].sum()) if "march.num_per_ray" in det else 0
        n_hit = int(det["march.num_per_ray"].shape[0]) if "march.num_per_ray" in det else 0
        K = int(vb["t"].shape[0]) if vb.get("type") == "packed" else 0
        return M + n_hit * sum(nf[:-1]), K, bool(out["ray_tested"].get("rays_coherent", False))

    def _size(self, grow=1.0):
        need_m, need_k, coh = self._probe()
        if self.coherent is None:
            self.coherent = coh
        floor = 4096 + 8 * min(self.n_rays, 65536)
        m = int(max(need_m * self.slack, floor) * grow)
        k = int(max(need_k * self.slack, floor) * grow)
        self.march_cap = max(self.march_cap or 0, m)
        self.kept_cap = max(self.kept_cap or 0, k)

    def _run(self):
        if self.pre_hook is not None:
            self.pre_hook()
        if self.zero_grads:
            for p in self.model.parameters():
                if p.grad is not None:
                    p.grad.zero_()
        cv = getattr(self.model, "ctrl_var", None)
        if cv is not None and hasattr(cv, "mix_weight"):
            if getattr(cv, "_w_dev", None) is None:
                cv._w_dev = torch.zeros((), device=self.device)
            cv._use_w_dev = True
        try:
            rendered, _, buffers = render_static(self.model, self.rays_o, self.rays_d, self.h_appear, near=self.near, far=self.far, march_cap=self.march_cap,
                                                 kept_cap=self.kept_cap, coherent=bool(self.coherent), with_rgb=self.with_rgb, with_normal=self.with_normal, cnt=self.cnt)
        finally:
            if cv is not None:
                cv._use_w_dev = False
        loss = None
        if self.loss_fn is not None:
            loss = self.loss_fn(rendered)
            if loss.requires_grad:
                loss.backward()
            loss = loss.detach()
        return rendered, buffers, loss

    def capture(self):
        if self.march_cap is None or self.kept_cap is None or self.coherent is None:
            self._size()
        if not self.use_graph:
            self.graph = None
            return self
        if not bool(self.rays_d.any()):
            raise RuntimeError("StaticFrame.capture: the input buffers hold no rays yet; call step(rays_o, rays_d, ...) or fill frame.rays_o / frame.rays_d first")
        was = L.KERNEL_TIMER.enabled
        L.KERNEL_TIMER.enabled = False
        import gc
        gc.collect()
        try:
            side = torch.cuda.Stream(device=self.device)
            side.wait_stream(torch.cuda.current_stream())
            with torch.cuda.stream(side):
                for _ in range(2):
                    self._run()
            torch.cuda.current_stream().wait_stream(side)
            torch.cuda.synchronize()
            g = torch.cuda.CUDAGraph()
            self._occ_captured = self.model.accel.occ.occ_grid
            with torch.cuda.graph(g, stream=side):
                self.rendered, self.buffers, self.loss = self._run()
            self.graph = g
            self.captures += 1
        finally:
            L.KERNEL_TIMER.enabled = was
        return self

    def step(self, rays_o, rays_d, rays_h_appear=None):
        self.rays_o.copy_(rays_o, non_blocking=True)
        self.rays_d.copy_(rays_d, non_blocking=True)
        if self.h_appear is not None and rays_h_appear is not None:
            self.h_appear.copy_(rays_h_appear, non_blocking=True)
        cv = getattr(self.model, "ctrl_var", None)
        if cv is not None and hasattr(cv, "mix_weight"):
            if getattr(cv, "_w_dev", None) is None:
                cv._w_dev = torch.zeros((), device=self.device)
            cv._w_dev.fill_(cv.mix_weight())
        if self.graph is None and (self.use_graph or self.march_cap is None):
            self.capture()
        if self.graph is not None:
            occ = self.model.accel.occ.occ_grid
            if self._occ_captured is not None and occ.data_ptr() != self._occ_captured.data_ptr():
                self._occ_captured.copy_(occ)
            self.graph.replay()
        else:
            self.rendered, self.buffers, self.loss = self._run()
        return self.loss

    def counts(self):
        c = self.cnt.tolist()
        return {k: c[v] for k, v in CNT_SLOTS.items()}

    def check(self, retry=True):
        if int(self.cnt[CNT_SLOTS["overflow"]]) == 0:
            return True
        self.march_cap = self.kept_cap = None
        self._size(grow=1.25)
        self.graph = None
        if self.use_graph:
            self.capture()
        if retry:
            if self.graph is not None:
                self.graph.replay()
            else:
                self.rendered, self.buffers, self.loss = self._run()
        return False

    def volume_buffer(self):
        return sliced_volume_buffer(self.buffers, self.cnt)
```

Measured before the change: 27.73.

## Recompute color MLP activations in backward instead of storing them; overlap wgmma groups

The forward now stores only the input activation tile (X) instead of four tiles (Z, X, Y1, Y2). The radiance and SDF backward kernels recompute Y1, Y2 and Z with extra wgmma GEMMs from X and staged weights and biases. The goal is to cut global memory traffic and activation storage. The mma helpers are split into issue and wait steps so that independent GEMMs and scalar work overlap, at the cost of extra tensor-core work and more shared memory.

New measurement: 27.82 (median of 6 runs). About the same (+0.3%).

```diff
diff --git a/neuralsim_b200/csrc/color_tc.cu b/neuralsim_b200/csrc/color_tc.cu
--- a/neuralsim_b200/csrc/color_tc.cu
+++ b/neuralsim_b200/csrc/color_tc.cu
@@ -56,12 +56,6 @@
         J0[gd] = a0;
         J1[gd] = a1;
     }
-}
-
-__device__ __forceinline__ void unpack8(const uint4 &q, float (&v)[8]) {
-    const __half2 *h = reinterpret_cast<const __half2 *>(&q);
-#pragma unroll
-    for (int i = 0; i < 4; ++i) { const float2 f = __half22float2(h[i]); v[2 * i] = f.x; v[2 * i + 1] = f.y; }
 }
 
 constexpr int kColorGatherU = 4;
@@ -248,9 +242,8 @@
 }
 
 __global__ void __launch_bounds__(kTile, kColorBwdCtasPerSM)
-k_color_rad_bwd(const ColorNetDev net, const uint8_t *__restrict__ Xt, const uint8_t *__restrict__ Y1t, const uint8_t *__restrict__ Y2t,
-                const float *__restrict__ rgb, const float *__restrict__ g_rgb, int64_t n, float *__restrict__ dh_out,
-                float *__restrict__ dR1, float *__restrict__ drb1, float *__restrict__ dR2, float *__restrict__ drb2,
+k_color_rad_bwd(const ColorNetDev net, const uint8_t *__restrict__ Xt, const float *__restrict__ rgb, const float *__restrict__ g_rgb, int64_t n,
+                float *__restrict__ dh_out, float *__restrict__ dR1, float *__restrict__ drb1, float *__restrict__ dR2, float *__restrict__ drb2,
                 float *__restrict__ dR3, float *__restrict__ drb3, const int64_t *__restrict__ n_dev) {
     n = eff_n(n, n_dev);
     constexpr int NE = 80;
@@ -261,7 +254,8 @@
     uint8_t *sXe = sY1 + kTile * NE * 2;
     uint8_t *sR2T = sXe + kTile * NE * 2;
     uint8_t *sR1h = sR2T + XW * XW * 2;
-    __shared__ float sR3[3][XW];
+    uint8_t *sR1 = sR1h + NF * XW * 2;
+    __shared__ float sR3[3][XW], srb1[XW], srb2[XW], sgy[kTile][3];
     __shared__ float sdb3[3];
     __shared__ __align__(8) uint64_t mbar_ld;
 
@@ -270,6 +264,9 @@
         const int i = e % XW, j = e / XW;
         const __half v = (j < net.rw && i < net.rw) ? net.R2[j * net.rw + i] : __float2half_rn(0.f);
         *reinterpret_cast<__half *>(sR2T + (j / 8) * (XW * 16) + i * 16 + (j % 8) * 2) = v;
+        const int rc = ref_col(i, net.n_appear);
+        const __half v1 = (j < net.rw && rc >= 0) ? net.R1[j * net.rin + rc] : __float2half_rn(0.f);
+        *reinterpret_cast<__half *>(sR1 + (i / 8) * (XW * 16) + j * 16 + (i % 8) * 2) = v1;
     }
     for (int e = tid; e < NF * XW; e += kTile) {
         const int k = e % NF, j = e / NF;
@@ -277,6 +274,8 @@
         *reinterpret_cast<__half *>(sR1h + (j / 8) * (NF * 16) + k * 16 + (j % 8) * 2) = v;
     }
     if (tid < XW) {
+        srb1[tid] = tid < net.rw ? __half2float(net.rb1[tid]) : 0.f;
+        srb2[tid] = tid < net.rw ? __half2float(net.rb2[tid]) : 0.f;
 #pragma unroll
         for (int k = 0; k < 3; ++k) sR3[k][tid] = tid < net.rw ? __half2float(net.R3[k * net.rw + tid]) : 0.f;
     }
@@ -296,15 +295,13 @@
     tc::fence_async_smem();
     __syncthreads();
     const uint32_t t_addr = tc::smem_u32(sT), y1_addr = tc::smem_u32(sY1), xe_addr = tc::smem_u32(sXe);
-    const uint32_t r2t_addr = tc::smem_u32(sR2T), r1h_addr = tc::smem_u32(sR1h);
+    const uint32_t r2t_addr = tc::smem_u32(sR2T), r1h_addr = tc::smem_u32(sR1h), r1_addr = tc::smem_u32(sR1);
     uint32_t ld_phase = 0;
     bool first_tile = true;
 
     const int64_t n_tiles = (n + kTile - 1) / kTile;
     auto fetch = [&](int64_t tile) {
-        tc::mbar_arrive_expect_tx(&mbar_ld, 3 * kTileBytes);
-        tc::tma_load_bulk(sT + 2 * kTileBytes, Y2t + tile * kTileBytes, kTileBytes, &mbar_ld);
-        tc::tma_load_bulk(sY1, Y1t + tile * kTileBytes, kTileBytes, &mbar_ld);
+        tc::mbar_arrive_expect_tx(&mbar_ld, kTileBytes);
         tc::tma_load_bulk(sXe, Xt + tile * kTileBytes, kTileBytes, &mbar_ld);
     };
     if (tid == 0 && (int64_t)blockIdx.x < n_tiles) fetch(blockIdx.x);
@@ -313,39 +310,75 @@
         const bool valid = i < n;
         tc::mbar_wait(&mbar_ld, ld_phase);
         ld_phase ^= 1;
-        float gy[3] = {0.f, 0.f, 0.f};
-        if (valid && g_rgb) {
+        {
+            float y[2][XW / 2];
+            tc::mma_m128_issue<64, 0, 0, XW / 16>(y, tc::kmajor(xe_addr, kTile), tc::kmajor(r1_addr, XW), false);
+            float gy[3] = {0.f, 0.f, 0.f};
+            if (valid && g_rgb) {
+#pragma unroll
+                for (int k = 0; k < 3; ++k) {
+                    const float yy = rgb[i * 3 + k];
+                    gy[k] = r16(r16(g_rgb[i * 3 + k]) * ((1.f - yy) * yy));
+                }
+            }
+            {
+                float e8[8] = {1.f, gy[0], gy[1], gy[2], 0.f, 0.f, 0.f, 0.f};
+                *reinterpret_cast<uint4 *>(sXe + 8 * kChunk + tid * 16) = tc::pack8_f16(e8);
+            }
 #pragma unroll
             for (int k = 0; k < 3; ++k) {
-                const float y = rgb[i * 3 + k];
-                gy[k] = r16(r16(g_rgb[i * 3 + k]) * ((1.f - y) * y));
-            }
-        }
-        {
-            float e8[8] = {1.f, gy[0], gy[1], gy[2], 0.f, 0.f, 0.f, 0.f};
-            *reinterpret_cast<uint4 *>(sXe + 8 * kChunk + tid * 16) = tc::pack8_f16(e8);
-        }
-#pragma unroll
-        for (int k = 0; k < 3; ++k) {
-            const float sgy = warp_sum(gy[k]);
-            if (lane == 0 && sgy != 0.f) atomicAdd(&sdb3[k], sgy);
-        }
-#pragma unroll 1
-        for (int c = 0; c < 8; ++c) {
-            float y2[8], d[8];
-            unpack8(*reinterpret_cast<const uint4 *>(sT + 2 * kTileBytes + c * kChunk + tid * 16), y2);
-#pragma unroll
-            for (int j = 0; j < 8; ++j) {
-                const float v = gy[0] * sR3[0][c * 8 + j] + gy[1] * sR3[1][c * 8 + j] + gy[2] * sR3[2][c * 8 + j];
-                d[j] = y2[j] > 0.f ? v : 0.f;
-            }
-            *reinterpret_cast<uint4 *>(sT + c * kChunk + tid * 16) = tc::pack8_f16(d);
+                sgy[tid][k] = gy[k];
+                const float sg = warp_sum(gy[k]);
+                if (lane == 0 && sg != 0.f) atomicAdd(&sdb3[k], sg);
+            }
+            tc::mma_wait();
+            tc::fence_frags(y);
+#pragma unroll
+            for (int h = 0; h < 2; ++h)
+#pragma unroll
+                for (int c = 0; c < XW / 8; ++c)
+#pragma unroll
+                    for (int r = 0; r < 2; ++r) {
+                        const int col = tc::frag_col(c);
+                        tc::st_pair_f16(sY1, tc::pair_off<kTile>(h * 64 + tc::frag_row(r), col), fmaxf(r16(y[h][4 * c + 2 * r] + srb1[col]), 0.f),
+                                        fmaxf(r16(y[h][4 * c + 2 * r + 1] + srb1[col + 1]), 0.f));
+                    }
+            tc::fence_async_smem();
+            __syncthreads();
+            tc::mma_m128<64, 0, 1, XW / 16>(y, tc::kmajor(y1_addr, kTile), tc::mnmajor(r2t_addr, XW), false);
+#pragma unroll
+            for (int h = 0; h < 2; ++h)
+#pragma unroll
+                for (int r = 0; r < 2; ++r) {
+                    const int row = h * 64 + tc::frag_row(r);
+                    const float g0 = sgy[row][0], g1 = sgy[row][1], g2 = sgy[row][2];
+#pragma unroll
+                    for (int c = 0; c < XW / 8; ++c) {
+                        const int col = tc::frag_col(c);
+                        const uint32_t off = tc::pair_off<kTile>(row, col);
+                        float y2[2], d[2];
+#pragma unroll
+                        for (int j = 0; j < 2; ++j) {
+                            y2[j] = fmaxf(r16(y[h][4 * c + 2 * r + j] + srb2[col + j]), 0.f);
+                            const float v = g0 * sR3[0][col + j] + g1 * sR3[1][col + j] + g2 * sR3[2][col + j];
+                            d[j] = y2[j] > 0.f ? v : 0.f;
+                        }
+                        tc::st_pair_f16(sT + 2 * kTileBytes, off, y2[0], y2[1]);
+                        tc::st_pair_f16(sT, off, d[0], d[1]);
+                    }
+                }
         }
         tc::fence_async_smem();
         __syncthreads();
         {
             float dy[2][XW / 2];
-            tc::mma_m128<64, 0, 0, XW / 16>(dy, tc::kmajor(t_addr, kTile), tc::kmajor(r2t_addr, XW), false);
+            tc::mma_m128_issue<64, 0, 0, XW / 16>(dy, tc::kmajor(t_addr, kTile), tc::kmajor(r2t_addr, XW), false);
+            tc::wgmma_commit();
+            tc::mma_m64_issue<NE, 1, 1, kTile / 16>(xa, tc::mnmajor(t_addr, kTile), tc::mnmajor(y1_addr, kTile), true);
+            tc::mma_m64_issue<8, 1, 1, kTile / 16>(x3, tc::mnmajor(t_addr + 2 * kTileBytes, kTile), tc::mnmajor(xe_addr + 8 * kChunk, kTile), true);
+            tc::wgmma_commit();
+            tc::wgmma_wait<1>();
+            tc::fence_frags(dy);
 #pragma unroll
             for (int h = 0; h < 2; ++h)
 #pragma unroll
@@ -360,10 +393,13 @@
         tc::fence_async_smem();
         __syncthreads();
         float dh[2][NF / 2];
-        tc::mma_m128<32, 0, 0, XW / 16>(dh, tc::kmajor(t_addr + kTileBytes, kTile), tc::kmajor(r1h_addr, NF), false);
-        tc::mma_m64<NE, 1, 1, kTile / 16>(xa, tc::mnmajor(t_addr, kTile), tc::mnmajor(y1_addr, kTile), true);
-        tc::mma_m64<NE, 1, 1, kTile / 16>(xb, tc::mnmajor(t_addr + kTileBytes, kTile), tc::mnmajor(xe_addr, kTile), true);
-        tc::mma_m64<8, 1, 1, kTile / 16>(x3, tc::mnmajor(t_addr + 2 * kTileBytes, kTile), tc::mnmajor(xe_addr + 8 * kChunk, kTile), true);
+        tc::mma_m128_issue<32, 0, 0, XW / 16>(dh, tc::kmajor(t_addr + kTileBytes, kTile), tc::kmajor(r1h_addr, NF), false);
+        tc::mma_m64_issue<NE, 1, 1, kTile / 16>(xb, tc::mnmajor(t_addr + kTileBytes, kTile), tc::mnmajor(xe_addr, kTile), true);
+        tc::mma_wait();
+        tc::fence_frags(dh);
+        tc::fence_frags(xa);
+        tc::fence_frags(xb);
+        tc::fence_frags(x3);
         first_tile = false;
         __syncthreads();
         if (tid == 0 && tile + gridDim.x < n_tiles) {
@@ -413,10 +449,10 @@
 }
 
 __global__ void __launch_bounds__(kTile, kColorBwdCtasPerSM)
-k_color_sdf_bwd(const PLMeta m, const __half *__restrict__ grid, const ColorNetDev net, const PointSrc ps, const uint8_t *__restrict__ Zt,
-                const uint8_t *__restrict__ Xt, const float *__restrict__ g_nab, const float *__restrict__ g_sdf, const float *__restrict__ dh_r,
-                int64_t n, int max_level, float *__restrict__ d_grid, float *__restrict__ d_W1, float *__restrict__ d_b1, float *__restrict__ d_W2,
-                float *__restrict__ d_b2, const int64_t *__restrict__ n_dev) {
+k_color_sdf_bwd(const PLMeta m, const __half *__restrict__ grid, const ColorNetDev net, const PointSrc ps, const uint8_t *__restrict__ Xt,
+                const float *__restrict__ g_nab, const float *__restrict__ g_sdf, const float *__restrict__ dh_r, int64_t n, int max_level,
+                float *__restrict__ d_grid, float *__restrict__ d_W1, float *__restrict__ d_b1, float *__restrict__ d_W2, float *__restrict__ d_b2,
+                const int64_t *__restrict__ n_dev) {
     n = eff_n(n, n_dev);
     constexpr int NX = 48;
     extern __shared__ uint8_t dyn_smem[];
@@ -430,14 +466,14 @@
     constexpr int kS = tc::acc_stride(2 * NF);
     float *stage = reinterpret_cast<float *>(sT);
     static_assert(kTile * kS * 4 <= 3 * kTileBytes, "the staged rows must fit in T");
-    __shared__ float sW2[HW], sdsdf[kTile];
+    __shared__ float sb1[HW], sW2[HW], sdsdf[kTile];
     __shared__ float sdb2;
     __shared__ __align__(8) uint64_t mbar_ld;
 
     const int tid = threadIdx.x, lane = tid & 31;
     stage_W1(net.dec, sW1, tid);
     stage_W1T(net.dec, sW1T, tid);
-    stage_decoder_vectors(net.dec, nullptr, sW2, nullptr, tid);
+    stage_decoder_vectors(net.dec, sb1, sW2, nullptr, tid);
     *reinterpret_cast<uint4 *>(sHe + 4 * kChunk + tid * 16) = make_uint4(0x00003C00u, 0, 0, 0);
     *reinterpret_cast<uint4 *>(sGe + 4 * kChunk + tid * 16) = make_uint4(0x00003C00u, 0, 0, 0);
     *reinterpret_cast<uint4 *>(sHe + 5 * kChunk + tid * 16) = make_uint4(0, 0, 0, 0);
@@ -462,37 +498,49 @@
 
     const int64_t n_tiles = (n + kTile - 1) / kTile;
     auto fetch = [&](int64_t tile) {
-        tc::mbar_arrive_expect_tx(&mbar_ld, kTileBytes + 4 * kChunk);
-        tc::tma_load_bulk(sZ, Zt + tile * kTileBytes, kTileBytes, &mbar_ld);
+        tc::mbar_arrive_expect_tx(&mbar_ld, 4 * kChunk);
         tc::tma_load_bulk(sHe, Xt + tile * kTileBytes, 4 * kChunk, &mbar_ld);
     };
     if (tid == 0 && (int64_t)blockIdx.x < n_tiles) fetch(blockIdx.x);
     for (int64_t tile = blockIdx.x; tile < n_tiles; tile += gridDim.x) {
         const int64_t i = tile * kTile + tid;
         const bool valid = i < n;
-        float xn[3], xs[3];
-        int64_t ray;
-        load_point(ps, ps.x == nullptr, i, valid, xn, xs, ray);
-        float gin[3] = {0.f, 0.f, 0.f};
-        if (valid && g_nab) {
-#pragma unroll
-            for (int d = 0; d < 3; ++d) gin[d] = g_nab[i * 3 + d] * net.fac[d] * 0.5f;
-        }
-        const float dsdf = (valid && g_sdf) ? g_sdf[i] : 0.f;
-        sdsdf[tid] = dsdf;
         tc::mbar_wait(&mbar_ld, ld_phase);
         ld_phase ^= 1;
-#pragma unroll 1
-        for (int c = 0; c < 8; ++c) {
-            float z[8], uu[8];
-            unpack8(*reinterpret_cast<const uint4 *>(sZ + c * kChunk + tid * 16), z);
-#pragma unroll
-            for (int j = 0; j < 8; ++j) {
-                float a, s;
-                softplus_as(z[j], spk, a, s);
-                uu[j] = sW2[c * 8 + j] * s;
-            }
-            *reinterpret_cast<uint4 *>(sT + kTileBytes + c * kChunk + tid * 16) = tc::pack8_f16(uu);
+        float xs[3], gin[3] = {0.f, 0.f, 0.f}, dsdf;
+        {
+            float z[2][HW / 2];
+            tc::mma_m128_issue<64, 0, 0, NF / 16>(z, tc::kmajor(he_addr, kTile), tc::kmajor(w1_addr, HW), false);
+            float xn[3];
+            int64_t ray;
+            load_point(ps, ps.x == nullptr, i, valid, xn, xs, ray);
+            if (valid && g_nab) {
+#pragma unroll
+                for (int d = 0; d < 3; ++d) gin[d] = g_nab[i * 3 + d] * net.fac[d] * 0.5f;
+            }
+            dsdf = (valid && g_sdf) ? g_sdf[i] : 0.f;
+            sdsdf[tid] = dsdf;
+            tc::mma_wait();
+            tc::fence_frags(z);
+#pragma unroll
+            for (int h = 0; h < 2; ++h)
+#pragma unroll
+                for (int c = 0; c < HW / 8; ++c)
+#pragma unroll
+                    for (int r = 0; r < 2; ++r) {
+                        const int col = tc::frag_col(c);
+                        const uint32_t off = tc::pair_off<kTile>(h * 64 + tc::frag_row(r), col);
+                        float zz[2], uu[2];
+#pragma unroll
+                        for (int j = 0; j < 2; ++j) {
+                            zz[j] = r16(z[h][4 * c + 2 * r + j] + sb1[col + j]);
+                            float a, s;
+                            softplus_as(zz[j], spk, a, s);
+                            uu[j] = sW2[col + j] * s;
+                        }
+                        tc::st_pair_f16(sZ, off, zz[0], zz[1]);
+                        tc::st_pair_f16(sT + kTileBytes, off, uu[0], uu[1]);
+                    }
         }
 #pragma unroll 4
         for (uint32_t p = 0; p < 16; ++p) {
@@ -513,8 +561,12 @@
         float gfr[2][NF / 2];
         {
             float du[2][HW / 2];
-            tc::mma_m128<64, 0, 0, NF / 16>(du, tc::kmajor(ge_addr, kTile), tc::kmajor(w1_addr, HW), false);
-            tc::mma_m128<32, 0, 0, HW / 16>(gfr, tc::kmajor(t_addr + kTileBytes, kTile), tc::kmajor(w1t_addr, NF), false);
+            tc::mma_m128_issue<64, 0, 0, NF / 16>(du, tc::kmajor(ge_addr, kTile), tc::kmajor(w1_addr, HW), false);
+            tc::wgmma_commit();
+            tc::mma_m128_issue<32, 0, 0, HW / 16>(gfr, tc::kmajor(t_addr + kTileBytes, kTile), tc::kmajor(w1t_addr, NF), false);
+            tc::wgmma_commit();
+            tc::wgmma_wait<1>();
+            tc::fence_frags(du);
 #pragma unroll
             for (int h = 0; h < 2; ++h)
 #pragma unroll
@@ -545,13 +597,18 @@
         tc::fence_async_smem();
         __syncthreads();
         float dhz[2][NF / 2];
-        tc::mma_m128<32, 0, 0, HW / 16>(dhz, tc::kmajor(t_addr, kTile), tc::kmajor(w1t_addr, NF), false);
-        tc::mma_m64<NX, 1, 1, kTile / 16>(wacc, tc::mnmajor(t_addr, kTile), tc::mnmajor(he_addr, kTile), true);
-        tc::mma_m64<NF, 1, 1, kTile / 16>(*reinterpret_cast<float(*)[NF / 2]>(wacc), tc::mnmajor(t_addr + kTileBytes, kTile), tc::mnmajor(ge_addr, kTile), true);
-        tc::mma_m64<8, 1, 1, kTile / 16>(vacc, tc::mnmajor(t_addr + 2 * kTileBytes, kTile), tc::mnmajor(ge_addr + 4 * kChunk, kTile), true);
-        first_tile = false;
+        tc::mma_m128_issue<32, 0, 0, HW / 16>(dhz, tc::kmajor(t_addr, kTile), tc::kmajor(w1t_addr, NF), false);
+        tc::mma_m64_issue<NX, 1, 1, kTile / 16>(wacc, tc::mnmajor(t_addr, kTile), tc::mnmajor(he_addr, kTile), true);
+        tc::mma_m64_issue<8, 1, 1, kTile / 16>(vacc, tc::mnmajor(t_addr + 2 * kTileBytes, kTile), tc::mnmajor(ge_addr + 4 * kChunk, kTile), true);
         const float dsum = warp_sum(dsdf);
         if (lane == 0 && dsum != 0.f) atomicAdd(&sdb2, dsum);
+        tc::mma_wait();
+        tc::fence_frags(gfr);
+        tc::fence_frags(dhz);
+        tc::fence_frags(wacc);
+        tc::fence_frags(vacc);
+        tc::mma_m64<NF, 1, 1, kTile / 16>(*reinterpret_cast<float(*)[NF / 2]>(wacc), tc::mnmajor(t_addr + kTileBytes, kTile), tc::mnmajor(ge_addr, kTile), true);
+        first_tile = false;
         __syncthreads();
         if (tid == 0 && tile + gridDim.x < n_tiles) {
             tc::fence_async_smem();
@@ -655,7 +712,7 @@
     if (n == 0) return 0;
     NSB_REQUIRE(meta && params_half && net && sdf && nablas && rgb && view_dirs, "nsb_fused_color_fwd: NULL argument");
     NSB_REQUIRE(x || (rays_o && rays_d && t), "nsb_fused_color_fwd: need x or (rays_o, rays_d, t)");
-    NSB_REQUIRE((act_z && act_x && act_y1 && act_y2) || (!act_z && !act_x && !act_y1 && !act_y2), "nsb_fused_color_fwd: pass all four activation buffers or none");
+    NSB_REQUIRE(act_x || (!act_z && !act_y1 && !act_y2), "nsb_fused_color_fwd: act_z, act_y1 and act_y2 are written only alongside act_x");
     PLMeta m;
     ColorNetDev d;
     if (int rc = make_net(net, meta, &m, &d, "nsb_fused_color_fwd")) return rc;
@@ -678,7 +735,7 @@
                                    void *stream) {
     const DevCounts dn = take_counts();
     if (n == 0) return 0;
-    NSB_REQUIRE(meta && params_half && net && act_z && act_x && act_y1 && act_y2 && rgb && dh_scratch, "nsb_fused_color_bwd: NULL argument");
+    NSB_REQUIRE(meta && params_half && net && act_x && rgb && dh_scratch, "nsb_fused_color_bwd: NULL argument");
     NSB_REQUIRE(d_grid && d_W1 && d_b1 && d_W2 && d_b2 && d_R1 && d_rb1 && d_R2 && d_rb2 && d_R3 && d_rb3, "nsb_fused_color_bwd: NULL gradient buffer");
     NSB_REQUIRE(x || (rays_o && rays_d && t), "nsb_fused_color_bwd: need x or (rays_o, rays_d, t)");
     PLMeta m;
@@ -687,12 +744,11 @@
     cudaStream_t s = (cudaStream_t)stream;
     const float *dh = nullptr;
     if (g_rgb) {
-        constexpr int kSmemR = 3 * kTileBytes + 2 * kTile * 80 * 2 + XW * XW * 2 + NF * XW * 2 + 1024;
+        constexpr int kSmemR = 3 * kTileBytes + 2 * kTile * 80 * 2 + 2 * XW * XW * 2 + NF * XW * 2 + 1024;
         opt_in_smem(k_color_rad_bwd, kSmemR);
         if (int rc = require_ctas_per_sm(k_color_rad_bwd, kTile, kSmemR, kColorBwdCtasPerSM, "nsb_fused_color_bwd(radiance)")) return rc;
-        k_color_rad_bwd<<<persistent_grid(n_tiles(n), kColorBwdCtasPerSM), kTile, kSmemR, s>>>(d, (const uint8_t *)act_x, (const uint8_t *)act_y1,
-                                                                                               (const uint8_t *)act_y2, rgb, g_rgb, n, dh_scratch, d_R1,
-                                                                                               d_rb1, d_R2, d_rb2, d_R3, d_rb3, dn.a);
+        k_color_rad_bwd<<<persistent_grid(n_tiles(n), kColorBwdCtasPerSM), kTile, kSmemR, s>>>(d, (const uint8_t *)act_x, rgb, g_rgb, n, dh_scratch,
+                                                                                               d_R1, d_rb1, d_R2, d_rb2, d_R3, d_rb3, dn.a);
         if (int rc = check_launch("nsb_fused_color_bwd(radiance)")) return rc;
         dh = dh_scratch;
     }
@@ -700,7 +756,7 @@
     opt_in_smem(k_color_sdf_bwd, kSmemS);
     if (int rc = require_ctas_per_sm(k_color_sdf_bwd, kTile, kSmemS, kColorBwdCtasPerSM, "nsb_fused_color_bwd(sdf)")) return rc;
     const PointSrc ps{x, rays_o, rays_d, t, ridx};
-    k_color_sdf_bwd<<<persistent_grid(n_tiles(n), kColorBwdCtasPerSM), kTile, kSmemS, s>>>(m, (const __half *)params_half, d, ps, (const uint8_t *)act_z, (const uint8_t *)act_x,
+    k_color_sdf_bwd<<<persistent_grid(n_tiles(n), kColorBwdCtasPerSM), kTile, kSmemS, s>>>(m, (const __half *)params_half, d, ps, (const uint8_t *)act_x,
                                                                           g_nablas, g_sdf, dh, n, max_level < 0 ? -1 : max_level, d_grid, d_W1, d_b1, d_W2, d_b2, dn.a);
     return check_launch("nsb_fused_color_bwd(sdf)");
 }
diff --git a/neuralsim_b200/csrc/tc_util.cuh b/neuralsim_b200/csrc/tc_util.cuh
--- a/neuralsim_b200/csrc/tc_util.cuh
+++ b/neuralsim_b200/csrc/tc_util.cuh
@@ -86,14 +86,24 @@
 __device__ __forceinline__ void wgmma_fence() { asm volatile("wgmma.fence.sync.aligned;" ::: "memory"); }
 __device__ __forceinline__ void wgmma_commit() { asm volatile("wgmma.commit_group.sync.aligned;" ::: "memory"); }
 __device__ __forceinline__ void wgmma_wait_all() { asm volatile("wgmma.wait_group.sync.aligned 0;" ::: "memory"); }
+template <int Pending>
+__device__ __forceinline__ void wgmma_wait() { asm volatile("wgmma.wait_group.sync.aligned %0;" ::"n"(Pending) : "memory"); }
 __device__ __forceinline__ void fence_operand(float &r) { asm volatile("" : "+f"(r)::"memory"); }
 
-template <int N, int TA, int TB, int KSTEPS>
-__device__ __forceinline__ void mma_m128(float (&d)[2][N / 2], const Operand &a, const Operand &b, bool accumulate) {
-#pragma unroll
-    for (int h = 0; h < 2; ++h)
-#pragma unroll
-        for (int i = 0; i < N / 2; ++i) fence_operand(d[h][i]);
+template <int K>
+__device__ __forceinline__ void fence_frags(float (&d)[K]) {
+#pragma unroll
+    for (int i = 0; i < K; ++i) fence_operand(d[i]);
+}
+template <int K>
+__device__ __forceinline__ void fence_frags(float (&d)[2][K]) {
+    fence_frags(d[0]);
+    fence_frags(d[1]);
+}
+
+template <int N, int TA, int TB, int KSTEPS>
+__device__ __forceinline__ void mma_m128_issue(float (&d)[2][N / 2], const Operand &a, const Operand &b, bool accumulate) {
+    fence_frags(d);
     wgmma_fence();
 #pragma unroll
     for (int h = 0; h < 2; ++h)
@@ -101,27 +111,33 @@
         for (int ks = 0; ks < KSTEPS; ++ks)
             Wgmma<N, TA, TB>::mma(d[h], make_desc(a.addr + h * 8 * a.sbo + ks * a.kstep, a.lbo, a.sbo), make_desc(b.addr + ks * b.kstep, b.lbo, b.sbo),
                                   (ks > 0 || accumulate) ? 1u : 0u);
-    wgmma_commit();
-    wgmma_wait_all();
-#pragma unroll
-    for (int h = 0; h < 2; ++h)
-#pragma unroll
-        for (int i = 0; i < N / 2; ++i) fence_operand(d[h][i]);
-}
-
-template <int N, int TA, int TB, int KSTEPS>
-__device__ __forceinline__ void mma_m64(float (&d)[N / 2], const Operand &a, const Operand &b, bool accumulate) {
-#pragma unroll
-    for (int i = 0; i < N / 2; ++i) fence_operand(d[i]);
+}
+template <int N, int TA, int TB, int KSTEPS>
+__device__ __forceinline__ void mma_m64_issue(float (&d)[N / 2], const Operand &a, const Operand &b, bool accumulate) {
+    fence_frags(d);
     wgmma_fence();
 #pragma unroll
     for (int ks = 0; ks < KSTEPS; ++ks)
         Wgmma<N, TA, TB>::mma(d, make_desc(a.addr + ks * a.kstep, a.lbo, a.sbo), make_desc(b.addr + ks * b.kstep, b.lbo, b.sbo),
                               (ks > 0 || accumulate) ? 1u : 0u);
+}
+__device__ __forceinline__ void mma_wait() {
     wgmma_commit();
     wgmma_wait_all();
-#pragma unroll
-    for (int i = 0; i < N / 2; ++i) fence_operand(d[i]);
+}
+
+template <int N, int TA, int TB, int KSTEPS>
+__device__ __forceinline__ void mma_m128(float (&d)[2][N / 2], const Operand &a, const Operand &b, bool accumulate) {
+    mma_m128_issue<N, TA, TB, KSTEPS>(d, a, b, accumulate);
+    mma_wait();
+    fence_frags(d);
+}
+
+template <int N, int TA, int TB, int KSTEPS>
+__device__ __forceinline__ void mma_m64(float (&d)[N / 2], const Operand &a, const Operand &b, bool accumulate) {
+    mma_m64_issue<N, TA, TB, KSTEPS>(d, a, b, accumulate);
+    mma_wait();
+    fence_frags(d);
 }
 
 __device__ __forceinline__ int frag_row(int i) { return (threadIdx.x >> 5) * 16 + ((threadIdx.x & 31) >> 2) + 8 * i; }
diff --git a/neuralsim_b200/fields/fused_color.py b/neuralsim_b200/fields/fused_color.py
--- a/neuralsim_b200/fields/fused_color.py
+++ b/neuralsim_b200/fields/fused_color.py
@@ -21,8 +21,8 @@
         x = torch.empty(n, 3, dtype=torch.float32, device=dev)
         acts = None
         if keep:
-            acts = torch.empty(4, int(L.lib().nsb_color_tile_bytes(L.c_i64(n))), dtype=torch.uint8, device=dev)
-        ap = [L.ptr(acts[k]) if keep else None for k in range(4)]
+            acts = torch.empty(int(L.lib().nsb_color_tile_bytes(L.c_i64(n))), dtype=torch.uint8, device=dev)
+        ap = [None, L.ptr(acts) if keep else None, None, None]
         with L.KERNEL_TIMER.time("fused_color_fwd", n):
             L.check(L.lib().nsb_fused_color_fwd(meta.c_ref, L.ptr(grid16, "f16"), ctypes.byref(net), None, L.ptr(rays_o, "f32"), L.ptr(rays_d, "f32"),
                                                 L.ptr(ridx, "i64"), L.ptr(t, "f32"), L.ptr(view_dirs, "f32"), L.ptr(h_appear, "f32", allow_none=True),
@@ -58,8 +58,8 @@
         dh = torch.empty(n, 32, dtype=torch.float32, device=dev)
         with L.KERNEL_TIMER.time("fused_color_bwd", n):
             L.check(L.lib().nsb_fused_color_bwd(meta.c_ref, L.ptr(grid16, "f16"), ctypes.byref(net), None, L.ptr(rays_o, "f32"), L.ptr(rays_d, "f32"),
-                                                L.ptr(ridx, "i64"), L.ptr(t, "f32"), L.c_i64(n), L.c_i32(ctx.max_level), L.ptr(acts[0]), L.ptr(acts[1]),
-                                                L.ptr(acts[2]), L.ptr(acts[3]), L.ptr(rgb), L.ptr(g_sdf, allow_none=True), L.ptr(g_nab, allow_none=True),
+                                                L.ptr(ridx, "i64"), L.ptr(t, "f32"), L.c_i64(n), L.c_i32(ctx.max_level), None, L.ptr(acts), None, None,
+                                                L.ptr(rgb), L.ptr(g_sdf, allow_none=True), L.ptr(g_nab, allow_none=True),
                                                 L.ptr(g_rgb, allow_none=True), L.ptr(dh), *[L.ptr(g) for g in grads], L.stream_ptr()),
                     "fused_color_bwd")
         return (None,) * 7 + tuple(grads)
diff --git a/neuralsim_b200/graphics/neus_static.py b/neuralsim_b200/graphics/neus_static.py
--- a/neuralsim_b200/graphics/neus_static.py
+++ b/neuralsim_b200/graphics/neus_static.py
@@ -168,8 +168,8 @@
         nab = torch.empty(n, 3, dtype=torch.float32, device=dev)
         rgb = torch.empty(n, 3, dtype=torch.float32, device=dev)
         x = torch.empty(n, 3, dtype=torch.float32, device=dev)
-        acts = torch.empty(4, int(L.lib().nsb_color_tile_bytes(L.c_i64(n))), dtype=torch.uint8, device=dev) if keep_acts else None
-        ap = [L.ptr(acts[k]) if keep_acts else None for k in range(4)]
+        acts = torch.empty(int(L.lib().nsb_color_tile_bytes(L.c_i64(n))), dtype=torch.uint8, device=dev) if keep_acts else None
+        ap = [None, L.ptr(acts) if keep_acts else None, None, None]
         P = L.ptr
         with L.KERNEL_TIMER.time("fused_color_fwd", n):
             _call(L.lib().nsb_fused_color_fwd, "fused_color_fwd", st.cnt, CNT_SLOTS["kept"], None,
@@ -205,7 +205,7 @@
         with L.KERNEL_TIMER.time("fused_color_bwd", n):
             _call(L.lib().nsb_fused_color_bwd, "fused_color_bwd", st.cnt, CNT_SLOTS["kept"], None,
                   st.meta.c_ref, P(st.grid16, "f16"), ctypes.byref(st.net), None, P(st.rays_o, "f32"), P(st.rays_d, "f32"), P(ctx.ridx, "i64"),
-                  P(ctx.t, "f32"), L.c_i64(n), L.c_i32(st.ml), P(acts[0]), P(acts[1]), P(acts[2]), P(acts[3]), P(rgb), P(g_sdf, allow_none=True),
+                  P(ctx.t, "f32"), L.c_i64(n), L.c_i32(st.ml), None, P(acts), None, None, P(rgb), P(g_sdf, allow_none=True),
                   P(g_nab, allow_none=True), P(g_rgb, allow_none=True), P(dh), *[P(g) for g in grads], L.stream_ptr())
         return (None,) * 6 + tuple(grads)
 
```
